# paninski-lab/deepgraphpose

Measured on AMD Instinct MI355X. Metric: frames_per_sec, higher is better.
Workload: dtype f32

## Files before the change

### deepgraphpose_amd/_lib.py

```python
from __future__ import annotations

import ctypes as C
import os

_HERE = os.path.dirname(os.path.abspath(__file__))
LIB_PATH = os.environ.get("DGP_HIP_LIB") or os.path.join(_HERE, "libdgp_hip.so")


class DgpNetDesc(C.Structure):
    _fields_ = [("depth", C.c_int32), ("num_joints", C.c_int32), ("in_h", C.c_int32), ("in_w", C.c_int32),
                ("max_batch", C.c_int32), ("with_locref", C.c_int32), ("mean_pixel", C.c_float * 3),
                ("bn_eps", C.c_float)]


class DgpTensorView(C.Structure):
    _fields_ = [("name", C.c_char_p), ("data", C.POINTER(C.c_float)), ("ndim", C.c_int32),
                ("shape", C.c_int64 * 4)]


class DgpLossDesc(C.Structure):
    _fields_ = [(n, C.c_int32) for n in ("nt", "H", "W", "nj", "nl", "n_visible", "n_hidden", "gm2", "gm3",
                                          "gauss_len", "huber")] + \
               [(n, C.c_float) for n in ("gamma", "lengthscale", "stride", "wn_visible", "wn_hidden",
                                         "locref_loss_weight", "n_frames_total", "n_visible_frames_total")] + \
# ... 8 lines not shown
class DgpJpegInfo(C.Structure):
    _fields_ = [(n, C.c_int32) for n in ("width", "height", "ncomp", "sampling", "mcus_x", "mcus_y")] + \
               [("blocks_x", C.c_int32 * 3), ("blocks_y", C.c_int32 * 3), ("blocks", C.c_int32 * 3)] + \
               [(n, C.c_int32) for n in ("total_blocks", "restart_interval", "reserved")] + [("scan_offset", C.c_int64)]


class DgpConvDesc(C.Structure):
    _fields_ = [(n, C.c_int32) for n in (
        "N", "H", "W", "Cin", "Cout", "KH", "KW", "stride", "rate", "pad_t", "pad_l", "Ho", "Wo", "relu",
        "res_stride", "res_H", "res_W")]


class DgpConvPlan(C.Structure):
    _fields_ = [(n, C.c_int32) for n in (
        "tile", "family", "mode", "cs", "dma", "deep", "ah2", "oh2", "h1", "lds", "mtiles", "ntiles", "grid",
        "tail_ksplit", "n_main", "st_gn", "st_mc", "st_mb", "n_cu")] + [("kernel_name", C.c_char * 32)]


_vp, _i32, _f32, _sz = C.c_void_p, C.c_int32, C.c_float, C.c_size_t
SYMBOLS = {
    "dgp_version": (C.c_int, []),
    "dgp_tuning_build": (C.c_int, []),
    "dgp_crc32c": (C.c_uint32, [C.c_void_p, C.c_size_t, C.c_uint32]),
    "dgp_last_error": (C.c_char_p, []),
    "dgp_net_create": (C.c_int, [C.POINTER(DgpNetDesc), C.POINTER(_vp)]),
    "dgp_net_destroy": (None, [_vp]),
    "dgp_net_set_input_size": (C.c_int, [_vp, _i32, _i32]),
    "dgp_dlc_loss_fwd_bwd": (C.c_int, [_vp, _vp, _vp, _vp, _vp, _vp, _i32, _i32, _i32, _i32, C.c_float, _i32, _vp, _vp, _vp,
                                       _vp, _sz, _vp]),
    "dgp_net_load_weights": (C.c_int, [_vp, C.POINTER(DgpTensorView), _i32]),
    "dgp_net_workspace_bytes": (C.c_int, [_vp, _i32, C.POINTER(_sz)]),
    "dgp_net_output_dims": (C.c_int, [_vp] + [C.POINTER(_i32)] * 4),
    "dgp_net_stats": (C.c_int, [_vp, _i32, C.POINTER(_i32), C.POINTER(C.c_double)]),
    "dgp_forward": (C.c_int, [_vp, _vp, _i32, _vp, _sz, _vp, _vp, _vp, _vp]),
    "dgp_soft_argmax": (C.c_int, [_vp, _i32, _i32, _i32, _i32, _f32, _i32, _vp, _vp, _vp, _vp, _vp]),
    "dgp_soft_argmax_locref": (C.c_int, [_vp, _vp, _i32, _i32, _i32, _i32, _f32, _i32, _vp, _vp, _vp, _vp, _vp, _vp]),
    "dgp_hard_argmax": (C.c_int, [_vp, _vp, _i32, _i32, _i32, _i32, _vp, _vp, _vp, _vp]),
    "dgp_pmap_threshold": (C.c_int, [_vp, _i32, _i32, _i32, _i32, _f32, _vp, _vp]),
    "dgp_infer": (C.c_int, [_vp, _vp, _i32, _vp, _sz, _f32, _i32, _vp, _vp, _vp, _vp, _vp]),
    "dgp_infer_packed": (C.c_int, [_vp, _vp, _i32, _vp, _sz, _f32, _i32, _vp, _vp, _vp]),
    "dgp_infer_packed_locref": (C.c_int, [_vp, _vp, _i32, _vp, _sz, _f32, _i32, _i32, _vp, _vp, _vp, _vp]),
    "dgp_net_profile_begin": (C.c_int, [_vp, _i32]),
    "dgp_net_profile_end": (C.c_int, [_vp, C.POINTER(_i32), C.POINTER(_i32)]),
    "dgp_net_profile_launch": (C.c_int, [_vp, _i32, C.c_char_p, _i32, C.POINTER(C.c_double), C.POINTER(C.c_double)]),
    "dgp_loss_scratch_bytes": (C.c_int, [C.POINTER(DgpLossDesc), C.POINTER(_sz)]),
    "dgp_loss_fwd_bwd": (C.c_int, [C.POINTER(DgpLossDesc)] + [_vp] * 18 + [_sz, _vp]),
    "dgp_trainer_create": (C.c_int, [_vp, C.POINTER(_vp)]),
    "dgp_trainer_destroy": (None, [_vp]),
    "dgp_trainer_num_tensors": (C.c_int, [_vp, C.POINTER(_i32), C.POINTER(C.c_int64), C.POINTER(C.c_int64)]),
    "dgp_trainer_tensor_info": (C.c_int, [_vp, _i32, C.c_char_p, _i32, C.POINTER(C.c_int64), C.POINTER(C.c_int64),
                                          C.POINTER(_i32)]),
    "dgp_trainer_buffer": (_vp, [_vp, _i32]),
    "dgp_trainer_upload": (C.c_int, [_vp, _i32, C.c_int64, _vp, C.c_int64]),
    "dgp_trainer_download": (C.c_int, [_vp, _i32, C.c_int64, _vp, C.c_int64]),
    "dgp_trainer_workspace_bytes": (C.c_int, [_vp, _i32, C.POINTER(_sz)]),
    "dgp_trainer_sync_weights": (C.c_int, [_vp, _vp]),
    "dgp_train_forward": (C.c_int, [_vp, _vp, _i32, _vp, _sz, C.POINTER(_vp), C.POINTER(_vp), _vp]),
    "dgp_train_backward": (C.c_int, [_vp, _i32, _vp, _sz, _vp, _vp, _vp]),
    "dgp_sgd_momentum_clip": (C.c_int, [_vp, _f32, _f32, _f32, C.POINTER(_f32), _vp]),
    "dgp_adam_clip": (C.c_int, [_vp, _f32, _f32, _f32, _f32, _f32, C.POINTER(_f32), _vp]),
    "dgp_packed_weight_floats": (_sz, [_i32, _i32, _i32, _i32]),
    "dgp_pack_conv_weights": (C.c_int, [_vp, _i32, _i32, _i32, _i32, _vp]),
    "dgp_conv2d": (C.c_int, [C.POINTER(DgpConvDesc), _vp, _vp, _vp, _vp, _vp, _vp, _vp]),
    "dgp_conv2d_ranged": (C.c_int, [C.POINTER(DgpConvDesc), _vp, _vp, _vp, _vp, _vp, _vp, _vp, _vp, _vp, _vp]),
    "dgp_conv2d_ranged_slab": (C.c_int, [C.POINTER(DgpConvDesc), _vp, _vp, _vp, _vp, _vp, _vp, _vp, _vp, _vp, _vp, _sz, _vp]),
    "dgp_conv2d_plan": (C.c_int, [C.POINTER(DgpConvDesc), _i32, _i32, _i32, _i32, _i32, _sz, _i32, _i32, C.POINTER(DgpConvPlan)]),
    "dgp_tensor_absmax": (C.c_int, [_vp, _sz, _vp, _vp]),
    "dgp_f32_to_h2": (C.c_int, [_vp, _sz, _i32, _vp, _vp]),
    "dgp_h2_to_f32": (C.c_int, [_vp, _sz, _i32, _vp, _vp]),
    "dgp_conv2d_h2": (C.c_int, [C.POINTER(DgpConvDesc), _vp, _i32, _vp, _vp, _vp, _vp, _vp, _i32, _i32, _vp, _i32, _i32, _vp, _vp, _vp]),
    "dgp_conv2d_h2_slab": (C.c_int, [C.POINTER(DgpConvDesc), _vp, _i32, _vp, _vp, _vp, _vp, _vp, _i32, _i32, _vp, _i32, _i32, _vp, _vp, _vp,
                                     _sz, _vp]),
    "dgp_net_set_tier": (C.c_int, [_vp, _i32]),
    "dgp_net_get_tier": (C.c_int, [_vp]),
    "dgp_f32_to_h1": (C.c_int, [_vp, _sz, _i32, _vp, _vp]),
    "dgp_h1_to_f32": (C.c_int, [_vp, _sz, _i32, _vp, _vp]),
    "dgp_conv2d_h1": (C.c_int, [C.POINTER(DgpConvDesc), _vp, _i32, _vp, _vp, _vp, _vp, _vp, _i32, _vp, _i32, _i32, _vp, _vp, _vp]),
    "dgp_chain_h2": (C.c_int, [_i32] * 9 + [_vp, _i32, _vp, _i32] + [_vp] * 6 + [_vp, _i32, _vp, _i32, _vp, _vp, _vp]),
    "dgp_unit_h2": (C.c_int, [_i32] * 7 + [_vp, _i32, _vp, _i32] + [_vp] * 3 + [_i32] + [_vp] * 6 + [_vp, _i32, _vp, _i32, _vp, _vp, _vp, _vp]),
    "dgp_chain_h1": (C.c_int, [_i32] * 9 + [_vp, _i32, _vp, _i32] + [_vp] * 6 + [_vp, _i32, _vp, _i32, _vp, _vp, _vp]),
    "dgp_unit_h1": (C.c_int, [_i32] * 7 + [_vp, _i32, _vp, _i32] + [_vp] * 3 + [_i32] + [_vp] * 6 + [_vp, _i32, _vp, _i32, _vp, _vp, _vp, _vp]),
    "dgp_chain_xkeep": (C.c_int, [_i32] * 11 + [_vp, _i32, _vp, _i32] + [_vp] * 6 + [_vp, _i32, _vp, _i32, _vp, _vp, _vp]),
    "dgp_unit_xkeep": (C.c_int, [_i32] * 9 + [_vp, _i32, _vp, _i32] + [_vp] * 3 + [_i32] + [_vp] * 6 + [_vp, _i32, _vp, _i32, _vp, _vp, _vp, _vp]),
    "dgp_net_range_status": (C.c_int, [_vp, C.POINTER(_i32), C.POINTER(_i32), _vp]),
    "dgp_net_recalibrate": (C.c_int, [_vp]),
    "dgp_net_reset_scales": (C.c_int, [_vp]),
    "dgp_net_copy_scales": (C.c_int, [_vp, _vp, _vp]),
    "dgp_net_widen": (C.c_int, [_vp]),
    "dgp_conv2d_wgrad": (C.c_int, [C.POINTER(DgpConvDesc), _vp, _vp, _vp, _vp, _vp, _vp, _vp]),
    "dgp_conv2d_wgrad_shadow": (C.c_int, [C.POINTER(DgpConvDesc), _vp, _vp, _vp, _vp, _vp, _vp, _vp, _vp, _vp, _vp]),
    "dgp_trainer_set_tier": (C.c_int, [_vp, C.c_int32]),
    "dgp_trainer_get_tier": (C.c_int, [_vp]),
    "dgp_trainer_grad_groups": (C.c_int, [_vp, C.c_int32, C.POINTER(C.c_int32), C.POINTER(C.c_int64), C.POINTER(C.c_int64)]),
    "dgp_trainer_grad_group_wait": (C.c_int, [_vp, C.c_int32, _vp]),
    "dgp_trainer_step_status": (C.c_int, [_vp, _vp, C.c_int32, C.POINTER(C.c_float), C.POINTER(C.c_float), C.POINTER(C.c_int32),
                                               C.POINTER(C.c_int32), _vp]),
    "dgp_trainer_fast_mode": (C.c_int, [_vp, C.c_int32]),
    "dgp_trainer_fast_status": (C.c_int, [_vp, C.POINTER(C.c_int32), C.POINTER(C.c_int32)]),
    "dgp_conv2d_dgrad_scratch_bytes": (_sz, [C.POINTER(DgpConvDesc)]),
    "dgp_conv2d_dgrad": (C.c_int, [C.POINTER(DgpConvDesc), _vp, _vp, _vp, _vp, _vp, _i32, _vp, _vp, _i32, _vp]),
    "dgp_h1_to_f32_pred": (C.c_int, [_vp, _sz, _vp, _vp, _vp, _vp]),
    "dgp_conv2d_wgrad_h1": (C.c_int, [C.POINTER(DgpConvDesc)] + [_vp] * 11),
    "dgp_conv2d_dgrad_h1": (C.c_int, [C.POINTER(DgpConvDesc), _vp, _vp, _vp, _vp, _vp, _i32] + [_vp] * 7),
    "dgp_stem_wgrad_h1": (C.c_int, [_vp] * 4 + [_i32] * 7 + [_vp] * 4),
    "dgp_heads_backward_h1": (C.c_int, [_vp] * 8 + [_i32] * 5 + [_vp] * 8),
    "dgp_motion_energy":(C.c_int, [_vp, C.c_int64, C.c_int32, _vp, _vp, _vp]),
    "dgp_maxpool_3x3s2_same": (C.c_int, [_vp, _i32, _i32, _i32, _i32, _vp, _vp]),
    "dgp_preprocess_u8": (C.c_int, [_vp, C.c_int64, C.POINTER(_f32), _vp, _vp]),
    "dgp_optical_flow_scratch_bytes": (C.c_int, [_i32, _i32, _i32, C.POINTER(DgpFlowParams), C.POINTER(_sz), C.POINTER(_i32)]),
    "dgp_optical_flow": (C.c_int, [_vp, _i32, _i32, _i32, C.POINTER(DgpFlowParams), _vp, _vp, _vp, _sz, _vp]),
    "dgp_resize_plan_size": (C.c_int, [_i32, _i32, C.POINTER(_i32)]),
    "dgp_resize_plan": (C.c_int, [_i32, _i32, _vp, _vp]),
    "dgp_resize_crop_u8": (C.c_int, [_vp, _i32, _i32, _i32, _i32, _i32, C.POINTER(_i32), _vp, _vp, _vp, _i32, _i32, _vp]),
    "dgp_resize_plan_size_f": (C.c_int, [_i32, _i32, _i32, C.POINTER(_i32)]),
    "dgp_resize_plan_f": (C.c_int, [_i32, _i32, _i32, _vp, _vp]),
    "dgp_window_resize_u8": (C.c_int, [_vp, _i32, _i32, _i32, _i32, _i32, _i32, _i32, _i32, _i32, _i32, _vp, _vp, _vp, _i32, _i32, _vp]),
    "dgp_target_maps": (C.c_int, [_vp, _vp, _vp, _vp, _i32, _i32, _i32, _i32, C.c_double, C.c_double, C.c_double, C.c_double, _i32,
                                  _vp, _vp, _vp, _vp, _vp]),
    "dgp_gather_frames_u8": (C.c_int, [_vp, C.c_int64, C.c_int64, _vp, _i32, _vp, _i32, C.c_int64, _vp, _vp]),
    "dgp_aug_affine_u8": (C.c_int, [_vp, _vp, _i32, _i32, C.POINTER(C.c_double), _vp]),
    "dgp_aug_blur3_u8": (C.c_int, [_vp, _vp, _i32, _i32, C.POINTER(_f32), _vp]),
    "dgp_aug_dropout_u8": (C.c_int, [_vp, _vp, _i32, _i32, _vp, _i32, _i32, _vp]),
    "dgp_aug_elastic_u8": (C.c_int, [_vp, _vp, _i32, _i32, _vp, _i32, _i32, _vp]),
    "dgp_aug_noise_u8": (C.c_int, [_vp, _vp, _i32, _i32, _f32, _i32, C.c_uint64, _vp]),
    "dgp_jpeg_probe": (C.c_int, [_vp, C.c_int64, C.POINTER(DgpJpegInfo)]),
    "dgp_jpeg_entropy_decode": (C.c_int, [_vp, C.c_int64, C.POINTER(DgpJpegInfo), _vp, _vp]),
    "dgp_jpeg_scratch_bytes": (_sz, [_i32, _i32, _i32, _i32]),
    "dgp_jpeg_reconstruct_u8": (C.c_int, [_vp, _vp, _i32, _i32, _i32, _i32, _vp, C.c_int64, _vp, _sz, _vp]),
    "dgp_jpeg_quality_tables": (C.c_int, [_i32, _vp]),
    "dgp_jpeg_encode_bound": (C.c_int64, [_i32, _i32, _i32]),
    "dgp_jpeg_entropy_encode": (C.c_int, [_vp, _i32, _i32, _i32, _vp, _vp, C.c_int64, C.POINTER(C.c_int64)]),
    "dgp_jpeg_forward_scratch_bytes": (_sz, [_i32, _i32, _i32, _i32]),
    "dgp_jpeg_forward_u8": (C.c_int, [_vp, _i32, _i32, _i32, C.c_int64, _i32, _vp, _vp, _i32, _i32, _vp, _vp, _sz, _vp]),
}

_lib = None


class DgpError(RuntimeError):
    pass


def load():
    global _lib
    if _lib is not None:
        return _lib
    if not os.path.exists(LIB_PATH):
        raise DgpError(
            "libdgp_hip.so not found at %s -- build it with `python -m deepgraphpose_amd.build` "
            "(hipcc --offload-arch=gfx950); deepgraphpose_amd has no CPU fallback" % LIB_PATH)
    try:
        import torch
    except ImportError:
        pass
    lib = C.CDLL(LIB_PATH)
    for name, (res, args) in SYMBOLS.items():
        fn = getattr(lib, name)
        fn.restype = res
        fn.argtypes = args
    _lib = lib
    return lib


def check(rc: int, what: str = ""):
    if rc != 0:
        msg = load().dgp_last_error()
# ... 2 lines not shown
```

### deepgraphpose_amd/arch.py

```python
from __future__ import annotations

import math
from dataclasses import dataclass
from typing import List, Tuple

BLOCKS = {
    50: [(64, 3, 2), (128, 4, 2), (256, 6, 2), (512, 3, 1)],
    101: [(64, 3, 2), (128, 4, 2), (256, 23, 2), (512, 3, 1)],
    152: [(64, 3, 2), (128, 8, 2), (256, 36, 2), (512, 3, 1)],
}

MEAN_PIXEL = (123.68, 116.779, 103.939)
BN_EPS = 1e-5


@dataclass
class UnitPlan:
    scope: str
    depth_in: int
    depth: int
    depth_bottleneck: int
    stride: int
    rate: int
    has_shortcut_conv: bool


def resnet_units(depth: int = 50, output_stride: int = 16) -> List[UnitPlan]:
    if depth not in BLOCKS:
        raise ValueError("unsupported resnet depth %r" % (depth,))
    name = "resnet_v1_%d" % depth
    target = output_stride // 4
    current_stride, rate = 1, 1
    units: List[UnitPlan] = []
    depth_in = 64
    for bi, (base, n_units, block_stride) in enumerate(BLOCKS[depth], start=1):
        for ui in range(1, n_units + 1):
            s = block_stride if ui == n_units else 1
            d_out = base * 4
            if current_stride == target:
                unit_stride, unit_rate = 1, rate
                rate *= s
            else:
                unit_stride, unit_rate = s, 1
                current_stride *= s
            units.append(UnitPlan(
                scope="%s/block%d/unit_%d/bottleneck_v1" % (name, bi, ui),
                depth_in=depth_in, depth=d_out, depth_bottleneck=base,
                stride=unit_stride, rate=unit_rate,
                has_shortcut_conv=(depth_in != d_out)))
            depth_in = d_out
    return units


def same_out(n: int, s: int) -> int:
    return -(-n // s)


def feature_hw(h: int, w: int, depth: int = 50) -> Tuple[int, int]:
    for _ in range(4):
        h, w = same_out(h, 2), same_out(w, 2)
    return h, w


def scoremap_hw(h: int, w: int, deconv_stride: int = 2) -> Tuple[int, int]:
    fh, fw = feature_hw(h, w)
    return fh * deconv_stride, fw * deconv_stride


def conv_macs_per_frame(h: int, w: int, depth: int = 50, nj: int = 4,
                        with_locref: bool = False) -> int:
    h1, w1 = same_out(h, 2), same_out(w, 2)
    macs = h1 * w1 * 7 * 7 * 3 * 64
    hh, ww = same_out(h1, 2), same_out(w1, 2)
    for u in resnet_units(depth):
        ho, wo = same_out(hh, u.stride), same_out(ww, u.stride)
        if u.has_shortcut_conv:
            macs += ho * wo * u.depth_in * u.depth
        macs += hh * ww * u.depth_in * u.depth_bottleneck
        macs += ho * wo * 9 * u.depth_bottleneck * u.depth_bottleneck
        macs += ho * wo * u.depth_bottleneck * u.depth
        hh, ww = ho, wo
    heads = nj * (3 if with_locref else 1)
    macs += hh * ww * 9 * 2048 * heads
    return macs


def launch_algorithmic_bytes(name: str, h: int, w: int, depth: int = 50, batch: int = 1, elem_bytes: float = 4.0) -> float:
    body = name.split("|")[0]
    if not body.startswith("conv:"):
        return 0.0
    if body.endswith("/conv1+pool"):
        h1, w1 = same_out(h, 2), same_out(w, 2)
        return float(batch * h * w * 3 + elem_bytes * batch * same_out(h1, 2) * same_out(w1, 2) * 64 + 4 * 7 * 7 * 3 * 64)
    toks = body[5:].split("+")
    units = {u.scope: (i, u) for i, u in enumerate(resnet_units(depth))}
    plan = resnet_units(depth)
    h1, w1 = same_out(h, 2), same_out(w, 2)
    hh, ww = same_out(h1, 2), same_out(w1, 2)
    geo = []
    for u in plan:
        ho, wo = same_out(hh, u.stride), same_out(ww, u.stride)
        geo.append((batch * hh * ww, batch * ho * wo))
        hh, ww = ho, wo
    convs = []
    for t in toks:
        if t == "shortcut":
            convs.append((convs[-1][0], "shortcut"))
            continue
        scope, _, which = t.rpartition("/")
        if scope not in units:
            return 0.0
        convs.append((units[scope][0], which))
    have = set(convs)
    total = 0.0
    for ui, which in convs:
        u = plan[ui]
        pin, pout = geo[ui]
        if which == "conv1":
            total += u.depth_in * u.depth_bottleneck
            total += pin * u.depth_bottleneck
            if (ui - 1, "conv3") not in have:
                total += pin * u.depth_in
        elif which == "conv2":
            total += 9 * u.depth_bottleneck * u.depth_bottleneck
            total += pin * u.depth_bottleneck
            if (ui, "conv3") not in have:
                total += pout * u.depth_bottleneck
        elif which == "conv3":
            total += u.depth_bottleneck * u.depth
            un = plan[ui + 1] if ui + 2 < len(plan) else None
            if (ui + 1, "conv1") in have and un is not None and un.stride == 2 and not un.has_shortcut_conv:
                pin_n, pout_n = geo[ui + 1]
                assert pin_n == pout
                total += pout_n * u.depth
            else:
                total += pout * u.depth
            if (ui, "conv2") not in have:
                total += pout * u.depth_bottleneck
            if (ui, "shortcut") in have:
                total += pin * u.depth_in
            elif u.has_shortcut_conv:
                total += pout * u.depth
            else:
                total += (pin if u.stride == 1 else pout) * u.depth
        elif which == "shortcut":
            total += u.depth_in * u.depth
            if (ui, "conv3") not in have:
                total += pin * u.depth_in + pout * u.depth
    return elem_bytes * total


def conv_algorithmic_bytes(h: int, w: int, depth: int = 50, batch: int = 1) -> dict:
    name = "resnet_v1_%d" % depth
    out = {}
    h1, w1 = same_out(h, 2), same_out(w, 2)
    out["conv:%s/conv1" % name] = 4.0 * (batch * h * w * 4 + batch * h1 * w1 * 64 + 7 * 7 * 4 * 64)
    hh, ww = same_out(h1, 2), same_out(w1, 2)
    for u in resnet_units(depth):
        ho, wo = same_out(hh, u.stride), same_out(ww, u.stride)
        pin, pout = batch * hh * ww, batch * ho * wo
        if u.has_shortcut_conv:
            out["conv:%s/shortcut" % u.scope] = 4.0 * (pin * u.depth_in + pout * u.depth + u.depth_in * u.depth)
        out["conv:%s/conv1" % u.scope] = 4.0 * (pin * u.depth_in + pin * u.depth_bottleneck + u.depth_in * u.depth_bottleneck)
        out["conv:%s/conv2" % u.scope] = 4.0 * (pin * u.depth_bottleneck + pout * u.depth_bottleneck +
                                                9 * u.depth_bottleneck * u.depth_bottleneck)
        res = pout * u.depth if u.has_shortcut_conv else (pin if u.stride == 1 else pout) * u.depth
        out["conv:%s/conv3" % u.scope] = 4.0 * (pout * u.depth_bottleneck + pout * u.depth + res + u.depth_bottleneck * u.depth)
        hh, ww = ho, wo
    return out
```

### deepgraphpose_amd/csrc/dgp_engine.h

```cpp
#pragma once
#include "../../include/dgp_hip.h"
#include "dgp_internal.h"

#include <cmath>
#include <cstdio>
#include <cstring>
#include <initializer_list>
#include <map>
#include <string>
#include <vector>

namespace dgp {
int fail(int code, const std::string& msg);
}
#define HIP_TRY(expr)                                                                          \
    do {                                                                                       \
        hipError_t _e = (expr);                                                                \
        if (_e != hipSuccess)                                                                  \
            return dgp::fail(DGP_ERR_HIP, std::string(#expr) + ": " + hipGetErrorString(_e));  \
    } while (0)

namespace dgp {

struct ConvLayer {
    std::string scope;
    int Cin = 0, Cout = 0, CoutP = 0, KH = 1, KW = 1, stride = 1, rate = 1;
    int nk = 0, ntaps = 1;
    bool has_bn = true, relu = false;
    float *d_w = nullptr, *d_scale = nullptr, *d_bias = nullptr;
    void* d_wh3 = nullptr;
    void* d_wh1 = nullptr;
    float *d_w_fused = nullptr, *d_bias_fused = nullptr;
    void* d_wh3_fused = nullptr;
    void* d_wh1_fused = nullptr;
    int nk_fused = 0, cin2 = 0;
    float* d_w_rows = nullptr;
    float* d_w_pw = nullptr;
    void* d_wh3_pw = nullptr;
    void* d_wh1_pw = nullptr;
    int coutp_pw = 0;
};

struct Unit {
    int sc = -1, c1 = -1, c2 = -1, c3 = -1;
    int stride = 1, rate = 1;
    int depth_in = 0, depth = 0, depth_bn = 0;
    int h = 0, w = 0, ho = 0, wo = 0, pb_h = 0, pb_w = 0;
};

struct ChainPlan {
    bool ok = false;
    int C = 0, C1 = 0, CIN2 = 0, res = 0;
    void* d_frags = nullptr;
    unsigned frag_bytes = 0;
    float *d_sc1 = nullptr, *d_bi1 = nullptr;
    int w3_exp = 0, w1_exp = 0;
    bool unit = false;
    int w2_exp = 0;
    unsigned head_bytes = 0;
    void* d_frags_h1 = nullptr;
    unsigned frag_bytes_h1 = 0, head_bytes_h1 = 0;
};
int build_chain_plan(ChainPlan& pl, int C, int C1, int CIN2, int res, const float* w3cat, const float* sc3, const float* bi3,
                     const float* w1, const float* sc1, const float* bi1, const float* w2 = nullptr, const float* sc2 = nullptr,
                     const float* bi2 = nullptr);
void free_chain_plan(ChainPlan& pl);

constexpr size_t TAIL_SLAB_FLOATS = (size_t)512 * 128 * 128;

int coutp_for(int cout);
int head_pw_coutp(int cpw);
int nk_for(int kh, int kw, int cin);
void tf_same(int n, int k, int s, int d, int* out, int* pad_before);
int pad_before_for(int n, int k, int stride, int rate, bool conv2d_same_explicit);

inline bool fits_descriptor(std::initializer_list<double> bytes) {
    for (double b : bytes) if (b > 4294967000.0) return false;
    return true;
}

inline int fill_conv_geometry(ConvArgs& a, const dgp_conv_desc& d, const char* too_big) {
    a.N = d.N; a.H = d.H; a.W = d.W; a.Cin = d.Cin; a.log2cin4 = ilog2(d.Cin / 4);
    a.Ho = d.Ho; a.Wo = d.Wo; a.Cout = d.Cout; a.CoutP = coutp_for(d.Cout);
    a.KH = d.KH; a.KW = d.KW; a.stride = d.stride; a.dil = d.rate; a.pad_t = d.pad_t; a.pad_l = d.pad_l;
    a.ntaps = d.KH * d.KW; a.nk = nk_for(d.KH, d.KW, d.Cin); a.M = d.N * d.Ho * d.Wo;
    a.res_s = d.res_stride; a.res_H = d.res_H; a.res_W = d.res_W; a.relu = d.relu;
    const double inb = (double)d.N * d.H * d.W * d.Cin * 4, outb = (double)a.M * d.Cout * 4;
    const double resb = a.res ? (double)d.N * d.res_H * d.res_W * d.Cout * 4 : 0.0;
    if (!fits_descriptor({inb, outb, resb})) return fail(DGP_ERR_INVALID, too_big);
    a.in_bytes = (unsigned)inb; a.out_bytes = (unsigned)outb; a.res_bytes = (unsigned)resb;
    a.w_bytes = (unsigned)((size_t)a.nk * 8 * a.CoutP * 16);
    return DGP_OK;
}
const char* const TOO_BIG = "activation tensor exceeds the 4 GiB buffer-descriptor range; lower the batch";

inline ConvArgs head_pointwise_args(const ConvLayer& l, const float* feat, int B, int h, int w, float* T, const float* feat_absmax,
                                    const float* w_absmax) {
    ConvArgs a{};
    a.in = feat; a.wpk = l.d_w_pw; a.wh3 = l.d_wh3_pw; a.out = T; a.in_absmax = feat_absmax; a.w_absmax = w_absmax;
    a.N = B; a.H = h; a.W = w; a.Cin = l.Cin; a.log2cin4 = ilog2(l.Cin / 4);
    a.Ho = h; a.Wo = w; a.Cout = l.coutp_pw; a.CoutP = l.coutp_pw;
    a.KH = 1; a.KW = 1; a.stride = 1; a.dil = 1; a.ntaps = 1; a.nk = nk_for(1, 1, l.Cin); a.M = B * h * w;
    a.in_bytes = (unsigned)((size_t)a.M * l.Cin * 4); a.out_bytes = (unsigned)((size_t)a.M * l.coutp_pw * 4);
    a.w_bytes = (unsigned)((size_t)a.nk * 8 * l.coutp_pw * 16); a.wh3_bytes = a.w_bytes;
    return a;
}

}

struct dgp_net {
    dgp_net_desc desc{};
    int device = 0;
    std::vector<dgp::ConvLayer> layers;
    int conv1 = -1, head_part = -1, head_locref = -1;
    std::vector<dgp::Unit> units;
    std::vector<dgp::ChainPlan> chains;
    bool loaded = false;
    int (*owner_sync)(void* owner, void* stream) = nullptr;
    void* owner = nullptr;
    int tier = 0;
    int h1 = 0, w1 = 0, hp = 0, wp = 0, fh = 0, fw = 0;
    float *d_wmax = nullptr, *d_amax = nullptr, *d_inmax = nullptr;
    float* tail_slab = nullptr;
    unsigned tail_slab_bytes = 0;
    bool wmax_valid = false;
    static constexpr int H2_NONE = (int)0x80000000;
    std::vector<int> act_exp;
    std::vector<char> unit_fuse_ok;
    bool h2_calibrated = false;
    int h2_head = 4;
    int h2_calibrations = 0;
    int *d_exps = nullptr, *d_flag = nullptr;
    const float* wmax(int li) const { return d_wmax ? d_wmax + (size_t)li * dgp::ABSMAX_SLOTS : nullptr; }
    float* amax(int li) const { return d_amax ? d_amax + (size_t)li * dgp::ABSMAX_SLOTS : nullptr; }
    bool prof_on = false, prof_in_infer = false;
    int prof_slots = 0, prof_used = 0, prof_launches = 0, prof_cursor = 0, prof_launches_used = 0;
    std::vector<hipEvent_t> prof_ev;
    std::vector<std::string> prof_names;
    std::vector<double> prof_flops;
    void prof_free() {
        for (auto e : prof_ev) (void)hipEventDestroy(e);
        prof_ev.clear();
    }
    ~dgp_net() {
        prof_free();
        for (auto& l : layers) {
            if (l.d_w) (void)hipFree(l.d_w);
            if (l.d_scale) (void)hipFree(l.d_scale);
            if (l.d_bias) (void)hipFree(l.d_bias);
            if (l.d_wh3) (void)hipFree(l.d_wh3);
            if (l.d_w_rows) (void)hipFree(l.d_w_rows);
            if (l.d_w_pw) (void)hipFree(l.d_w_pw);
            if (l.d_wh3_pw) (void)hipFree(l.d_wh3_pw);
            for (void* q : {l.d_wh1, l.d_wh1_fused, l.d_wh1_pw}) if (q) (void)hipFree(q);
            for (void* q : {(void*)l.d_w_fused, (void*)l.d_bias_fused, l.d_wh3_fused}) if (q) (void)hipFree(q);
        }
        for (auto& c : chains) dgp::free_chain_plan(c);
        for (float* q : {d_wmax, d_amax, d_inmax}) if (q) (void)hipFree(q);
        for (int* q : {d_exps, d_flag}) if (q) (void)hipFree(q);
    }
};
```

### deepgraphpose_amd/csrc/dgp_internal.h

```cpp
#pragma once
#include <hip/hip_runtime.h>
#include <stdint.h>
#include <stddef.h>
#include <stdlib.h>
#include <string.h>

namespace dgp {

constexpr int BK = 32;

struct ConvArgs {
    const float* in;
    const float* wpk;
    const float* scale;
    const float* bias;
    const float* res;
    const float* mask;
    float*       out;
    int N, H, W, Cin, log2cin4;
    int Ho, Wo, Cout, CoutP;
    int KH, KW, stride, dil, pad_t, pad_l;
    int ntaps, nk;
    int M;
    int res_s, res_H, res_W;
    int ksplit;
    long long split_stride;
    int up;
    int relu;
    int out_mode;
    int dc_nj;
    int mtiles, ntiles;
    int tap_minor;
    int stem;
    int tap_rows;
    float* slab;
    unsigned slab_bytes;
    int n_main, tail_ksplit;
    int epi_nt;
    int st_gn, st_mc, st_mb;
    const float* in2;
    const float* in2_absmax;
    unsigned in2_bytes;
    int cin_split;
    unsigned long long* dbg;
    unsigned in_bytes, w_bytes, res_bytes, out_bytes;
    const float* in_absmax;
    const float* w_absmax;
    const void*  wh3;
    unsigned     wh3_bytes;
    float*       out_absmax;
    int   in_fmt, out_fmt, res_fmt;
    float in_scale;
    float out_scale;
    float res_inv_scale;
    float*       shadow;
    const float* shadow_prev;
    int          shadow_fmt;
    const float* in_scale_dev;
    const float* out_scale_dev;
    const float* res_scale_dev;
    int mask_fmt;
};

constexpr int ABSMAX_SLOTS = 256;

enum TileCfg { TILE_128x128 = 0, TILE_128x64 = 1, TILE_64x64 = 2, TILE_128x32 = 3, TILE_128x128_W8 = 4, TILE_128x128_LS = 5, TILE_128x64_LS = 6, TILE_128x128_S6 = 7, TILE_128x128_S3 = 8, TILE_128x64_S6 = 9, TILE_128x128_S6K16 = 10, TILE_128x128_S3K16 = 11, TILE_128x128_S6K16W8 = 12, TILE_128x128_H3K16 = 13, TILE_128x128_H3K16W8 = 14, TILE_128x64_H3 = 15, TILE_128x128_H3K32 = 16 };

enum TileFamily { FAM_F32, FAM_LS, FAM_SPLIT };

struct SplitPath {
    int mode;
    bool pb;
    bool cs, dma, deep;
    bool ah2, oh2, h1;
    size_t lds;
};

struct ConvPlan {
    int tile;
    TileFamily family;
    bool wide;
    SplitPath path;
    int mtiles, ntiles;
    long long grid;
    int tail_ksplit, n_main;
    int st_gn, st_mc, st_mb;
};
hipError_t plan_conv(ConvArgs& a, int tile_cfg, int n_cu, ConvPlan& pl);
hipError_t launch_conv(const ConvArgs& a, int tile_cfg, hipStream_t s);
int        pick_tile(int M, int CoutP, int K, bool have_absmax = false);
hipError_t launch_pack_h3(const float* panel, int nk, int CoutP, const float* w_absmax, void* out, hipStream_t s);
hipError_t launch_pack_h1(const float* panel, int nk, int CoutP, const float* w_absmax, void* out, hipStream_t s);
hipError_t launch_f32_to_h1(const float* x, long long n_groups8, float scale, void* out, hipStream_t s);
hipError_t launch_h1_to_f32(const void* x, long long n_groups8, float inv_scale, float* out, hipStream_t s);
struct PackH3Desc { const float* panel; int nkg; int CoutP; const float* rng; void* out; };
hipError_t launch_pack_h3_all(const PackH3Desc* table_dev, int n, hipStream_t s);
hipError_t launch_pack_h1_all(const PackH3Desc* table_dev, int n, hipStream_t s);
hipError_t launch_absmax(const float* x, long long n, float* out_slots, hipStream_t s);
const char* conv_kernel_name(const ConvArgs& a, int tile_cfg);
hipError_t launch_reduce_slabs(const float* slabs, long long n, long long stride, int nsplit, float* out, hipStream_t s);
hipError_t launch_head_gather(const float* T, const float* bias, int B, int h, int w, int njt, int ldt, float* out, hipStream_t s);
hipError_t launch_maxpool(const float* x, int N, int H, int W, int C, float* y, hipStream_t s, float h2_scale = 0.f);
hipError_t launch_f32_to_h2(const float* x, long long n_groups8, float scale, void* out, hipStream_t s);
hipError_t launch_h2_to_f32(const void* x, long long n_groups8, float inv_scale, float* out, hipStream_t s);
hipError_t launch_h2_range_check(const float* amax_slots, const int* exps, int n_layers, int* flag, hipStream_t s);
hipError_t launch_stem_pool_fused(const unsigned char* frames, int B, int H, int W, const void* wcells, const float* w_absmax,
                                  const float* bn_scale, const float* bn_bias, float m0, float m1, float m2, float out_scale,
                                  float* out, float* out_absmax, hipStream_t s, int out_h1 = 0, const float* out_prev = nullptr,
                                  unsigned char* idx = nullptr);
hipError_t launch_preprocess(const uint8_t* f, long long npix, float m0, float m1, float m2,
                             float* out, hipStream_t s);
hipError_t launch_motion_energy(const uint8_t* frames, long long frame_bytes, int n_frames, const uint8_t* prev_frame,
                                unsigned long long* sums, hipStream_t s);
constexpr size_t SOFT_ARGMAX_LDS_LIMIT = 150 * 1024;
hipError_t launch_soft_argmax(const float* scmap, int B, int H, int W, int C, float gamma,
                              int gauss_len, float* mu, float* conf, int* idx, float* pmap,
                              hipStream_t s, int record_stride = 0);
hipError_t launch_soft_argmax_locref(const float* scmap, const float* locref, int B, int H, int W, int C, float gamma,
                                     int gauss_len, float* mu, float* conf, int* idx, float* offs, float* pmap,
                                     hipStream_t s, int record_stride = 0);
hipError_t launch_hard_argmax(const float* scmap, const float* locref, int B, int H, int W, int C,
                              int* idx, float* prob, float* offs, hipStream_t s, float* rec = nullptr, int record_stride = 0);
hipError_t launch_pmap_threshold(float* pmap, int B, int H, int W, int C, float th, float* mu, hipStream_t s);

struct LossArgs {
    const float* pred;
    const float* locref_pred;
    const float* mu;
    const float* targets;
    const float* locref_map;
    const float* locref_mask;
    const int* visible_marker; const int* hidden_marker; const int* visible_in_targets;
    const float* S0; const float* ws; const float* ws_max;
    float* dpred; float* dlocref;
    float* losses;
    float* t_all; float* dLdt; int* kind; float* stats; float* norm;
    int nt, H, W, nj, nl, n_v, n_h;
    int gm2, gm3, gauss_len, huber;
    float gamma, lengthscale, stride, hidden_scale, clique_scale, locref_weight;
    const float* vector_field; const float* wt_batch; float* wt_w;
    int use_wt, Hin, Win;
    float wt_max, temporal_scale;
};
constexpr size_t LOSS_LDS_LIMIT = 150 * 1024;
hipError_t launch_loss(const LossArgs& a, hipStream_t s);

struct DlcLossArgs {
    const float *pred, *part_targets, *part_weights;
    const float *locref_pred, *locref_targets, *locref_mask;
    float *dpred, *dlocref, *losses;
    double* acc;
    long long n_part, n_loc;
    float locref_loss_weight;
    int huber;
};
hipError_t launch_dlc_loss(const DlcLossArgs& a, hipStream_t s);

struct ChainArgs {
    const void* r2;
    const void* src2;
    void* xout;
    void* r1out;
    const void* wfrag;
    const float* sc1;
    const float* bi1;
    float post1, post2;
    float res_inv_scale, xout_scale, r1_scale;
    float* xout_absmax; float* r1_absmax;
    int M, HoWo, Wo, res_H, res_W;
    int ntiles;
    unsigned r2_bytes, src2_bytes, xout_bytes, r1_bytes, w_bytes;
    const void* r1in;
    unsigned r1in_bytes;
    int H, W, TY, TX;
    float post0, r2_scale;
    float* r2_absmax;
    int nt;
    int h1;
    int xkeep;
};
bool chain_supported(int C, int C1, int CIN2, int res);
int  chain_frags_per_chunk(int C, int C1, int CIN2, int planes = 2);
hipError_t launch_chain(const ChainArgs& a, int C, int C1, int CIN2, int res, hipStream_t s);
const char* chain_kernel_name(int C, int C1, int CIN2, int res);
bool unit_supported(int C, int C1, int CIN2, int res);
hipError_t launch_unit(const ChainArgs& a, int N, int C, int C1, int CIN2, int res, hipStream_t s);
hipError_t launch_chain_pack(const float* src, int n_chunks, int f1_pairs, int f2_pairs, float s1, float s2, void* out, hipStream_t s, int planes = 2);

inline int dgp_env(const char* name, int dflt) {
    const char* v = getenv(name);
    return v ? atoi(v) : dflt;
}
// ... 46 lines not shown
```

### deepgraphpose_amd/csrc/dgp_net.hip

```cpp
#include "dgp_engine.h"

using namespace dgp;

static thread_local std::string g_err;
namespace dgp {
int fail(int code, const std::string& msg) {
    g_err = msg;
    return code;
}

int coutp_for(int cout) {
    if (cout <= 32) return 32;
    if (cout <= 64) return 64;
    return round_up(cout, 128);
}
int head_pw_coutp(int cpw) { const int c = coutp_for(cpw); return c < 64 ? 64 : c; }
int nk_for(int kh, int kw, int cin) { return (kh * kw * (cin / 4) + 7) / 8; }

void tf_same(int n, int k, int s, int d, int* out, int* pad_before) {
    const int keff = (k - 1) * d + 1;
    *out = (n + s - 1) / s;
    int total = (*out - 1) * s + keff - n;
    if (total < 0) total = 0;
    *pad_before = total / 2;
// ... 19 lines not shown

int build_chain_plan(ChainPlan& pl, int C, int C1, int CIN2, int res, const float* w3cat, const float* sc3, const float* bi3,
                     const float* w1, const float* sc1, const float* bi1, const float* w2, const float* sc2, const float* bi2) {
    free_chain_plan(pl);
    if (!chain_supported(C, C1, CIN2, res)) return DGP_OK;
    const bool unit = w2 && unit_supported(C, C1, CIN2, res);
    const int C4 = 4 * C, KS1 = (C + CIN2) / 32, NJP = C4 / 32, NCB = C1 / 16;
    const int pairs = KS1 * 2 + NCB;
    const size_t chunk_f = (size_t)pairs * 512 + 256;
    const int KS2 = C / 32, NCB2 = C / 16, pairs2 = KS2 * NCB2;
    const size_t chunk2_f = (size_t)pairs2 * 512 + 256;
    std::vector<float> src((size_t)NJP * chunk_f, 0.f), src2(unit ? 9 * chunk2_f : 0, 0.f);
    float m3 = 0.f, m1 = 0.f, m2 = 0.f;
    for (size_t i = 0; i < (size_t)(C + CIN2) * C4; ++i) m3 = std::max(m3, fabsf(w3cat[i]));
    for (size_t i = 0; i < (size_t)C4 * C1; ++i) m1 = std::max(m1, fabsf(w1[i]));
    auto col_of = [](int cb, int i) { return 32 * (cb >> 1) + 8 * (i >> 2) + 4 * (cb & 1) + (i & 3); };
    for (int jp = 0; jp < NJP; ++jp) {
        float* ch = src.data() + (size_t)jp * chunk_f;
        for (int s = 0; s < KS1; ++s)
            for (int b = 0; b < 2; ++b) {
                float* f = ch + (size_t)(s * 2 + b) * 512;
                for (int ln = 0; ln < 64; ++ln) {
                    const int g = ln >> 4, i = ln & 15, col = 32 * jp + col_of(b, i);
                    for (int j = 0; j < 8; ++j) f[ln * 8 + j] = w3cat[(size_t)(32 * s + 8 * g + j) * C4 + col];
                }
            }
        for (int cb = 0; cb < NCB; ++cb) {
            float* f = ch + (size_t)(KS1 * 2 + cb) * 512;
            for (int ln = 0; ln < 64; ++ln) {
                const int g = ln >> 4, i = ln & 15, col = col_of(cb, i);
                for (int j = 0; j < 8; ++j) f[ln * 8 + j] = w1[(size_t)(32 * jp + 8 * g + j) * C1 + col];
            }
        }
        float* af = ch + (size_t)pairs * 512;
        for (int c = 0; c < 32; ++c) { af[c] = sc3 ? sc3[32 * jp + c] : 1.f; af[32 + c] = bi3 ? bi3[32 * jp + c] : 0.f; }
    }
    if (unit) {
        for (size_t i = 0; i < (size_t)9 * C * C; ++i) m2 = std::max(m2, fabsf(w2[i]));
        for (int t = 0; t < 9; ++t) {
            float* ch = src2.data() + (size_t)t * chunk2_f;
            for (int ks = 0; ks < KS2; ++ks)
                for (int cb = 0; cb < NCB2; ++cb) {
                    float* f = ch + (size_t)(ks * NCB2 + cb) * 512;
                    for (int ln = 0; ln < 64; ++ln) {
                        const int g = ln >> 4, i = ln & 15, col = col_of(cb, i);
                        for (int j = 0; j < 8; ++j) f[ln * 8 + j] = w2[((size_t)t * C + 32 * ks + 8 * g + j) * C + col];
                    }
                }
            float* af = ch + (size_t)pairs2 * 512;
            for (int c = 0; c < C; ++c) { af[c] = sc2 ? sc2[c] : 1.f; af[C + c] = bi2 ? bi2[c] : 0.f; }
        }
    }
    pl.C = C; pl.C1 = C1; pl.CIN2 = CIN2; pl.res = res; pl.unit = unit;
    pl.w3_exp = pow2_exp_for_max(m3); pl.w1_exp = pow2_exp_for_max(m1); pl.w2_exp = pow2_exp_for_max(m2);
    const int nf = chain_frags_per_chunk(C, C1, CIN2), nf2 = 2 * pairs2 + 1;
    const size_t head = unit ? (size_t)9 * nf2 * 1024 : 0;
    pl.frag_bytes = (unsigned)(head + (size_t)NJP * nf * 1024);
    pl.head_bytes = (unsigned)head;
    float *d_src = nullptr, *d_src2 = nullptr;
    HIP_TRY(hipMalloc(&d_src, src.size() * sizeof(float)));
    hipError_t e = hipMemcpy(d_src, src.data(), src.size() * sizeof(float), hipMemcpyHostToDevice);
    if (e == hipSuccess) e = hipMalloc(&pl.d_frags, pl.frag_bytes);
    if (e == hipSuccess && unit) e = hipMalloc(&d_src2, src2.size() * sizeof(float));
    if (e == hipSuccess && unit) e = hipMemcpy(d_src2, src2.data(), src2.size() * sizeof(float), hipMemcpyHostToDevice);
    if (e == hipSuccess && unit) e = launch_chain_pack(d_src2, 9, pairs2, 0, ldexpf(1.f, pl.w2_exp), 1.f, pl.d_frags, nullptr);
    if (e == hipSuccess) e = launch_chain_pack(d_src, NJP, KS1 * 2, NCB, ldexpf(1.f, pl.w3_exp), ldexpf(1.f, pl.w1_exp), (char*)pl.d_frags + head, nullptr);
    const int nf_h1 = chain_frags_per_chunk(C, C1, CIN2, 1), nf2_h1 = pairs2 + 1;
    const size_t head_h1 = unit ? (size_t)9 * nf2_h1 * 1024 : 0;
    pl.frag_bytes_h1 = (unsigned)(head_h1 + (size_t)NJP * nf_h1 * 1024);
    pl.head_bytes_h1 = (unsigned)head_h1;
    if (e == hipSuccess) e = hipMalloc(&pl.d_frags_h1, pl.frag_bytes_h1);
    if (e == hipSuccess && unit) e = launch_chain_pack(d_src2, 9, pairs2, 0, ldexpf(1.f, pl.w2_exp), 1.f, pl.d_frags_h1, nullptr, 1);
    if (e == hipSuccess) e = launch_chain_pack(d_src, NJP, KS1 * 2, NCB, ldexpf(1.f, pl.w3_exp), ldexpf(1.f, pl.w1_exp), (char*)pl.d_frags_h1 + head_h1, nullptr, 1);
    if (e == hipSuccess) e = hipDeviceSynchronize();
    (void)hipFree(d_src);
    if (d_src2) (void)hipFree(d_src2);
    if (e == hipSuccess) e = hipMalloc(&pl.d_sc1, C1 * sizeof(float));
    if (e == hipSuccess) e = hipMalloc(&pl.d_bi1, C1 * sizeof(float));
    std::vector<float> one(C1, 1.f), zero(C1, 0.f);
    if (e == hipSuccess) e = hipMemcpy(pl.d_sc1, sc1 ? sc1 : one.data(), C1 * sizeof(float), hipMemcpyHostToDevice);
    if (e == hipSuccess) e = hipMemcpy(pl.d_bi1, bi1 ? bi1 : zero.data(), C1 * sizeof(float), hipMemcpyHostToDevice);
    if (e != hipSuccess) { free_chain_plan(pl); return fail(DGP_ERR_HIP, std::string("chain plan: ") + hipGetErrorString(e)); }
    pl.ok = true;
    return DGP_OK;
}
}

namespace {

void pack_panels(const float* hwio, int KH, int KW, int Cin, int Cout, float* packed, int coutp = 0) {
    const int cin4 = Cin / 4, CoutP = coutp ? coutp : coutp_for(Cout), nk = nk_for(KH, KW, Cin);
    const size_t total = (size_t)nk * 8 * CoutP * 4;
    memset(packed, 0, total * sizeof(float));
    const int nchunks = KH * KW * cin4;
    for (int q = 0; q < nchunks; ++q) {
        const int tap = q / cin4, ch = (q % cin4) * 4;
        for (int e = 0; e < 4; ++e) {
            const float* src = hwio + ((size_t)tap * Cin + ch + e) * Cout;
            float* dst = packed + (size_t)q * CoutP * 4 + e;
            for (int co = 0; co < Cout; ++co) dst[(size_t)co * 4] = src[co];
        }
    }
}

}

static int add_layer(dgp_net* net, const std::string& scope, int cin, int cout, int k, int stride, int rate,
                     bool bn, bool relu) {
    ConvLayer l;
    l.scope = scope; l.Cin = cin; l.Cout = cout; l.KH = l.KW = k; l.stride = stride; l.rate = rate;
    l.CoutP = coutp_for(cout); l.nk = nk_for(k, k, cin); l.ntaps = k * k; l.has_bn = bn; l.relu = relu;
    net->layers.push_back(l);
    return (int)net->layers.size() - 1;
}

static void set_geometry(dgp_net* net, int in_h, int in_w) {
    int pb;
    net->desc.in_h = in_h; net->desc.in_w = in_w;
    net->h1 = (in_h + 1) / 2; net->w1 = (in_w + 1) / 2;
    tf_same(net->h1, 3, 2, 1, &net->hp, &pb); tf_same(net->w1, 3, 2, 1, &net->wp, &pb);
    int h = net->hp, w = net->wp;
    for (Unit& u : net->units) {
        u.h = h; u.w = w; tf_same(h, 3, u.stride, u.rate, &u.ho, &pb); tf_same(w, 3, u.stride, u.rate, &u.wo, &pb);
        u.pb_h = pad_before_for(h, 3, u.stride, u.rate, true); u.pb_w = pad_before_for(w, 3, u.stride, u.rate, true);
        h = u.ho; w = u.wo;
    }
    net->fh = h; net->fw = w;
}

extern "C" {

int dgp_version(void) { return DGP_ABI_VERSION; }

uint32_t dgp_crc32c(const void* data, size_t n, uint32_t crc) {
    static uint32_t tab[8][256];
    static bool init = false;
    if (!init) {
        for (uint32_t i = 0; i < 256; ++i) {
            uint32_t c = i;
            for (int k = 0; k < 8; ++k) c = (c & 1) ? (c >> 1) ^ 0x82F63B78u : c >> 1;
            tab[0][i] = c;
        }
        for (uint32_t i = 0; i < 256; ++i)
            for (int t = 1; t < 8; ++t) tab[t][i] = (tab[t - 1][i] >> 8) ^ tab[0][tab[t - 1][i] & 0xFF];
        init = true;
    }
    const uint8_t* p = (const uint8_t*)data;
    crc = ~crc;
    while (n >= 8) {
        uint32_t lo, hi;
        memcpy(&lo, p, 4);
        memcpy(&hi, p + 4, 4);
        lo ^= crc;
        crc = tab[7][lo & 0xFF] ^ tab[6][(lo >> 8) & 0xFF] ^ tab[5][(lo >> 16) & 0xFF] ^ tab[4][lo >> 24] ^
              tab[3][hi & 0xFF] ^ tab[2][(hi >> 8) & 0xFF] ^ tab[1][(hi >> 16) & 0xFF] ^ tab[0][hi >> 24];
        p += 8;
        n -= 8;
    }
    while (n--) crc = tab[0][(crc ^ *p++) & 0xFF] ^ (crc >> 8);
    return ~crc;
}
const char* dgp_last_error(void) { return g_err.c_str(); }
int dgp_tuning_build(void) {
#ifdef DGP_TUNING
    return 1;
#else
// ... 202 lines not shown
            HIP_TRY(hipMemcpy(l.d_w_rows, rows.data(), rows.size() * sizeof(float), hipMemcpyHostToDevice));
            if (!l.d_wh3) HIP_TRY(hipMalloc(&l.d_wh3, rows.size() * sizeof(float)));
            e = launch_pack_h3(l.d_w_rows, 7, l.CoutP, net->d_wmax + li * ABSMAX_SLOTS, l.d_wh3, nullptr);
            if (e != hipSuccess) return fail(DGP_ERR_HIP, std::string("stem weight cells: ") + hipGetErrorString(e));
        } else if (l.d_w_pw) {
            const int nkpw = nk_for(1, 1, 2048);
            float* wm = net->d_wmax + (nl + li) * ABSMAX_SLOTS;
            e = launch_absmax(l.d_w_pw, (long long)nkpw * 8 * l.coutp_pw * 4, wm, nullptr);
            if (e == hipSuccess) e = launch_pack_h3(l.d_w_pw, nkpw, l.coutp_pw, wm, l.d_wh3_pw, nullptr);
            if (e == hipSuccess && !l.d_wh1_pw) e = hipMalloc(&l.d_wh1_pw, (size_t)nkpw * 8 * l.coutp_pw * 8);
            if (e == hipSuccess) e = launch_pack_h1(l.d_w_pw, nkpw, l.coutp_pw, wm, l.d_wh1_pw, nullptr);
            if (e != hipSuccess) return fail(DGP_ERR_HIP, std::string("head pointwise panel: ") + hipGetErrorString(e));
        } else if (l.Cin >= 32 && l.CoutP % 64 == 0) {
            const size_t bytes = (size_t)l.nk * 8 * l.CoutP * 16;
            if (!l.d_wh3) HIP_TRY(hipMalloc(&l.d_wh3, bytes));
            e = launch_pack_h3(l.d_w, l.nk, l.CoutP, net->d_wmax + li * ABSMAX_SLOTS, l.d_wh3, nullptr);
            if (e == hipSuccess && (l.Cin % 64) == 0 && (l.nk % 2) == 0) {
                if (!l.d_wh1) e = hipMalloc(&l.d_wh1, bytes / 2);
                if (e == hipSuccess) e = launch_pack_h1(l.d_w, l.nk, l.CoutP, net->d_wmax + li * ABSMAX_SLOTS, l.d_wh1, nullptr);
            }
            if (e != hipSuccess) return fail(DGP_ERR_HIP, std::string("weight cells: ") + hipGetErrorString(e));
        }
    }
    for (const Unit& u : net->units) {
        if (u.sc < 0) continue;
        ConvLayer& l3 = net->layers[u.c3];
        const ConvLayer& ls = net->layers[u.sc];
        if (l3.KH != 1 || ls.KH != 1 || ls.stride != 1 || l3.Cin % 32 || ls.Cin % 32 || l3.Cout != ls.Cout) continue;
        const int c1 = l3.Cin, c2 = ls.Cin, co = l3.Cout;
        std::vector<float> w((size_t)(c1 + c2) * co), b(co);
        const std::vector<float>&w3 = keep_w[u.c3], &wsc = keep_w[u.sc], &s3 = keep_scale[u.c3], &ssc = keep_scale[u.sc];
        for (int k = 0; k < c1; ++k) for (int o = 0; o < co; ++o) w[(size_t)k * co + o] = w3[(size_t)k * co + o] * s3[o];
        for (int k = 0; k < c2; ++k) for (int o = 0; o < co; ++o) w[(size_t)(c1 + k) * co + o] = wsc[(size_t)k * co + o] * ssc[o];
        for (int o = 0; o < co; ++o) b[o] = keep_bias[u.c3][o] + keep_bias[u.sc][o];
        l3.nk_fused = (c1 + c2) / 32; l3.cin2 = c2;
        const size_t nfl = (size_t)l3.nk_fused * 8 * l3.CoutP * 4;
        std::vector<float> packed(nfl);
        pack_panels(w.data(), 1, 1, c1 + c2, co, packed.data());
        if (!l3.d_w_fused) HIP_TRY(hipMalloc(&l3.d_w_fused, nfl * sizeof(float)));
        if (!l3.d_bias_fused) HIP_TRY(hipMalloc(&l3.d_bias_fused, co * sizeof(float)));
        if (!l3.d_wh3_fused) HIP_TRY(hipMalloc(&l3.d_wh3_fused, nfl * sizeof(float)));
        HIP_TRY(hipMemcpy(l3.d_w_fused, packed.data(), nfl * sizeof(float), hipMemcpyHostToDevice));
        HIP_TRY(hipMemcpy(l3.d_bias_fused, b.data(), co * sizeof(float), hipMemcpyHostToDevice));
        float* wm = net->d_wmax + (nl + (size_t)u.c3) * ABSMAX_SLOTS;
        hipError_t e = launch_absmax(l3.d_w_fused, (long long)nfl, wm, nullptr);
        if (e == hipSuccess) e = launch_pack_h3(l3.d_w_fused, l3.nk_fused, l3.CoutP, wm, l3.d_wh3_fused, nullptr);
        if (e == hipSuccess && (c1 % 64) == 0 && (c2 % 64) == 0) {
            if (!l3.d_wh1_fused) e = hipMalloc(&l3.d_wh1_fused, nfl * 2);
            if (e == hipSuccess) e = launch_pack_h1(l3.d_w_fused, l3.nk_fused, l3.CoutP, wm, l3.d_wh1_fused, nullptr);
        }
        if (e != hipSuccess) return fail(DGP_ERR_HIP, std::string("fused shortcut panel: ") + hipGetErrorString(e));
    }
    for (auto& c : net->chains) free_chain_plan(c);
    net->chains.assign(net->units.size(), ChainPlan());
    for (size_t ui = 0; ui + 1 < net->units.size(); ++ui) {
        const Unit &u = net->units[ui], &un = net->units[ui + 1];
        const ConvLayer &l3 = net->layers[u.c3], &l1 = net->layers[un.c1];
        if (l3.KH != 1 || l1.KH != 1 || l1.stride != 1 || l3.Cout != 4 * l3.Cin || l1.Cin != l3.Cout) continue;
        const int C = l3.Cin, C1 = l1.Cout;
        static const bool wide_env = (dgp_tune("DGP_CHAIN_WIDE", 0) != 0);
        if (C > 128 && !wide_env) continue;
        const ConvLayer& l2 = net->layers[u.c2];
        const bool c2_plain = l2.KH == 3 && l2.stride == 1 && l2.rate == 1 && l2.Cin == C && l2.Cout == C;
        const float *w2 = c2_plain ? keep_w[u.c2].data() : nullptr, *s2 = c2_plain ? keep_scale[u.c2].data() : nullptr,
                    *b2 = c2_plain ? keep_bias[u.c2].data() : nullptr;
        int rc2;
        if (u.sc >= 0) {
            const ConvLayer& ls = net->layers[u.sc];
            if (ls.stride != 1 || u.stride != 1 || !l3.d_w_fused) continue;
            const int c2 = ls.Cin, co = l3.Cout;
            std::vector<float> w((size_t)(C + c2) * co), b(co);
            const std::vector<float>&w3 = keep_w[u.c3], &wsc = keep_w[u.sc], &s3 = keep_scale[u.c3], &ssc = keep_scale[u.sc];
            for (int k = 0; k < C; ++k) for (int o = 0; o < co; ++o) w[(size_t)k * co + o] = w3[(size_t)k * co + o] * s3[o];
            for (int k = 0; k < c2; ++k) for (int o = 0; o < co; ++o) w[(size_t)(C + k) * co + o] = wsc[(size_t)k * co + o] * ssc[o];
            for (int o = 0; o < co; ++o) b[o] = keep_bias[u.c3][o] + keep_bias[u.sc][o];
            rc2 = build_chain_plan(net->chains[ui], C, C1, c2, 0, w.data(), nullptr, b.data(), keep_w[un.c1].data(),
                                   keep_scale[un.c1].data(), keep_bias[un.c1].data(), w2, s2, b2);
        } else {
            rc2 = build_chain_plan(net->chains[ui], C, C1, 0, u.stride == 1 ? 1 : 2, keep_w[u.c3].data(), keep_scale[u.c3].data(),
                                   keep_bias[u.c3].data(), keep_w[un.c1].data(), keep_scale[un.c1].data(), keep_bias[un.c1].data(), w2, s2, b2);
        }
        if (rc2) return rc2;
    }
    HIP_TRY(hipDeviceSynchronize());
    net->wmax_valid = true;
    net->loaded = true;
    net->h2_calibrated = false;
    net->h2_head = 4;
    net->act_exp.assign(net->layers.size(), 0);
    net->unit_fuse_ok.assign(net->units.size(), 1);
    if (!net->d_exps) HIP_TRY(hipMalloc(&net->d_exps, net->layers.size() * sizeof(int)));
    if (!net->d_flag) { HIP_TRY(hipMalloc(&net->d_flag, 2 * sizeof(int))); HIP_TRY(hipMemset(net->d_flag, 0, 2 * sizeof(int))); }
    return DGP_OK;
}

}

namespace {

constexpr int HEAD_KSPLIT_MAX = 8;

struct Plan {
    size_t off_p0, off_c1, off_x0, off_x1, off_sc, off_r1, off_r2, off_scmap, off_locref, off_slabs, off_tail, total;
};

size_t align256(size_t x) { return (x + 255) / 256 * 256; }

Plan make_plan(const dgp_net* net, int B) {
    const dgp_net_desc& d = net->desc;
    size_t p0 = (size_t)B * d.in_h * d.in_w * 4;
    size_t c1 = (size_t)B * net->h1 * net->w1 * 64;
    size_t x = (size_t)B * net->hp * net->wp * 64, sc = 0, r1 = 0, r2 = 0;
    for (const Unit& u : net->units) {
        r1 = std::max(r1, (size_t)B * u.h * u.w * u.depth_bn);
        r2 = std::max(r2, (size_t)B * u.ho * u.wo * u.depth_bn);
        x = std::max(x, (size_t)B * u.ho * u.wo * u.depth);
        if (u.sc >= 0) sc = std::max(sc, (size_t)B * u.ho * u.wo * u.depth);
    }
    r1 = r2 = std::max(r1, r2);
    Plan p{};
    size_t o = 0;
    auto take = [&](size_t nfloats) { size_t r = o; o += align256(nfloats * sizeof(float)); return r; };
    p.off_p0 = take(p0); p.off_c1 = take(c1); p.off_x0 = take(x); p.off_x1 = take(x); p.off_sc = take(sc);
    p.off_r1 = take(r1); p.off_r2 = take(r2);
    p.off_scmap = take((size_t)B * 4 * net->fh * net->fw * d.num_joints);
    p.off_locref = take((size_t)B * 4 * net->fh * net->fw * 2 * d.num_joints);
    p.off_slabs = take((size_t)HEAD_KSPLIT_MAX * B * 4 * net->fh * net->fw * 2 * d.num_joints);
    p.off_tail = take(TAIL_SLAB_FLOATS);
    p.total = o;
    return p;
}

struct ProfScope {
    dgp_net* net; hipStream_t s; int li;
    ProfScope(dgp_net* n, hipStream_t st, const std::string& name, double flops) : net(n), s(st), li(-1) {
        if (!net->prof_on || net->prof_used >= net->prof_slots) return;
        li = net->prof_cursor++;
        if (li >= net->prof_launches) { li = -1; return; }
        if (net->prof_used == 0) { net->prof_names[li] = name; net->prof_flops[li] = flops; }
        (void)hipEventRecord(net->prof_ev[((size_t)net->prof_used * net->prof_launches + li) * 2], s);
    }
    ~ProfScope() {
        if (li >= 0) (void)hipEventRecord(net->prof_ev[((size_t)net->prof_used * net->prof_launches + li) * 2 + 1], s);
    }
};

double conv_flops_of(const ConvLayer& l, int M, bool is_head) {
    if (is_head) return 2.0 * M * 9.0 * l.Cin * (l.Cout / 4);
    const int cin = (l.KH == 7) ? 3 : l.Cin;
    return 2.0 * M * (double)l.KH * l.KW * cin * l.Cout;
}

struct H2Spec { int in_fmt = 0, in_exp = 0, out_fmt = 0, out_exp = 0, res_fmt = 0, res_exp = 0; };

void apply_h2(ConvArgs& a, const H2Spec& h) {
    a.in_fmt = h.in_fmt; a.out_fmt = h.out_fmt; a.res_fmt = h.res_fmt;
    a.in_scale = ldexpf(1.f, h.in_exp); a.out_scale = ldexpf(1.f, h.out_exp); a.res_inv_scale = ldexpf(1.f, -h.res_exp);
}

struct ConvCall {
    const float* in = nullptr;
    int H = 0, W = 0, Ho = 0, Wo = 0, pad_t = 0, pad_l = 0;
    const float* res = nullptr;
    int res_s = 0, res_H = 0, res_W = 0;
    bool relu = true;
    int out_mode = 0, dc_nj = 0;
// ... 174 lines not shown
        HIP_TRY(hipStreamSynchronize(s));
        HIP_TRY(hipMemcpy(host, net->amax(li), sizeof host, hipMemcpyDeviceToHost));
        *mx = 0.f;
        for (float v : host) *mx = (v > *mx || v != v) ? v : *mx;
        return DGP_OK;
    }
    template <class Launch>
    int layer(int li, Launch&& launch, int forced_exp = dgp_net::H2_NONE, bool* forced_ok = nullptr) const {
        int r = launch();
        if (r || !calib) return r;
        float mx = 0.f;
        if ((r = read_range(li, &mx))) return r;
        int e = exp_for(mx);
        if (forced_exp != dgp_net::H2_NONE) {
            const bool ok = forced_exp <= e + net->h2_head - 1 && forced_exp >= e - 6;
            if (forced_ok) *forced_ok = ok;
            if (ok) e = forced_exp;
        }
        if (e != net->act_exp[li]) {
            net->act_exp[li] = e;
            HIP_TRY(hipMemsetAsync(net->amax(li), 0, ABSMAX_SLOTS * sizeof(float), s));
            r = launch();
        }
        return r;
    }
    H2Spec spec(int in_exp, int out_li, bool with_res = false, int res_exp = 0) const {
        H2Spec q;
        q.in_fmt = FMT; q.in_exp = in_exp; q.out_fmt = FMT; q.out_exp = net->act_exp[out_li]; q.res_fmt = with_res ? FMT : 0; q.res_exp = res_exp;
        return q;
    }
    bool can_fuse(int ui) const {
        const Unit& u = net->units[ui];
        return fuse_on && u.sc >= 0 && net->layers[u.c3].d_w_fused && u.stride == 1 && u.ho == u.h && u.wo == u.w && net->layers[u.c3].CoutP % 64 == 0;
    }
    int conv(int li, const ConvCall& call) const { return run_conv(net, net->layers[li], B, call, s); }
};

int fwd_context(FwdCtx& c, dgp_net* net, const uint8_t* frames, int B, char* ws, const Plan& pl, hipStream_t s) {
    static const bool h2_env = (dgp_env("DGP_H2", 1) != 0);
    static const bool head_pw = (dgp_tune("DGP_HEAD_PW", 1) != 0);
    static const bool fuse_env = (dgp_env("DGP_FUSE_SHORTCUT", 1) != 0);
    static const bool cells_env = (dgp_tune("DGP_PRESPLIT_WEIGHTS", 1) != 0);
    static const bool stem_fused_env = (dgp_tune("DGP_STEM_FUSED", 1) != 0);
    static const bool chain_env = (dgp_env("DGP_CHAIN", 1) != 0);
    static const bool chain_h1_env = (dgp_env("DGP_CHAIN_H1", 1) != 0);
    static const bool unit_env = (dgp_tune("DGP_UNIT", 1) != 0);
    static const bool xsub_env = (dgp_env("DGP_XOUT_SUBSAMPLE", 1) != 0);
    c = FwdCtx{};
    c.net = net; c.s = s; c.B = B; c.frames = frames;
    c.P0 = (float*)(ws + pl.off_p0); c.C1 = (float*)(ws + pl.off_c1); c.X[0] = (float*)(ws + pl.off_x0); c.X[1] = (float*)(ws + pl.off_x1);
    c.SC = (float*)(ws + pl.off_sc); c.R1 = (float*)(ws + pl.off_r1); c.R2 = (float*)(ws + pl.off_r2);
    c.scmap_ws = (float*)(ws + pl.off_scmap); c.slabs = (float*)(ws + pl.off_slabs);
    const ConvLayer& lpart = net->layers[net->head_part];
    const ConvLayer* lloc = net->head_locref < 0 ? nullptr : &net->layers[net->head_locref];
    c.f16_mode = conv_mode() == ConvMode::F16x3 || conv_mode() == ConvMode::F16;
    c.head_pw = head_pw; c.unit_on = unit_env; c.xsub_on = xsub_env;
    c.fuse_on = fuse_env && conv_mode() != ConvMode::F32 && net->wmax_valid;
    c.tier = net->tier; c.FMT = c.tier ? 2 : 1;
    c.h2 = h2_env && cells_env && c.f16_mode && head_pw && net->wmax_valid && net->d_exps && lpart.d_wh3_pw && (!lloc || lloc->d_wh3_pw) &&
           net->act_exp.size() == net->layers.size();
    if (c.tier) {
        bool ok = c.h2 && lpart.d_wh1_pw && (!lloc || lloc->d_wh1_pw);
        for (const Unit& u : net->units) {
            ok = ok && net->layers[u.c1].d_wh1 && net->layers[u.c2].d_wh1 && net->layers[u.c3].d_wh1 && (u.sc < 0 || net->layers[u.sc].d_wh1);
            if (u.sc >= 0 && net->layers[u.c3].d_w_fused && !net->layers[u.c3].d_wh1_fused) ok = false;
        }
        if (!ok) return fail(DGP_ERR_STATE, "dgp_forward: the 16-bit tier needs the H2 engine's switches at their defaults (DGP_H2, DGP_PRESPLIT_WEIGHTS, "
                                            "DGP_HEAD_PW, DGP_CONV_MODE unset or f16) and weights loaded by dgp_net_load_weights");
    }
    c.calib = c.h2 && !net->h2_calibrated;
    const ConvLayer& lstem = net->layers[net->conv1];
    c.stem_fused = c.h2 && (stem_fused_env || c.tier) && lstem.d_wh3 && lstem.d_w_rows && lstem.CoutP == 64 && lstem.d_scale && lstem.d_bias;
    if (c.tier && !c.stem_fused) return fail(DGP_ERR_STATE, "dgp_forward: the 16-bit tier needs the fused root block");
    c.chain_tier = chain_env && (!c.tier || chain_h1_env);
    c.chain_on = c.h2 && !c.calib && c.chain_tier && net->chains.size() == net->units.size();
    return DGP_OK;
}

int forward_root(FwdCtx& c) {
    dgp_net* net = c.net;
    const dgp_net_desc& d = net->desc;
    const ConvLayer& lstem = net->layers[net->conv1];
    int rc;
    if (c.stem_fused) {
        rc = c.layer(net->conv1, [&] {
            ProfScope ps(net, c.s, "conv:" + lstem.scope + "+pool|stem_pool_fused", conv_flops_of(lstem, c.B * net->h1 * net->w1, false));
            hipError_t e2 = launch_stem_pool_fused(c.frames, c.B, d.in_h, d.in_w, lstem.d_wh3, net->wmax(net->conv1), lstem.d_scale, lstem.d_bias,
                                                   d.mean_pixel[0], d.mean_pixel[1], d.mean_pixel[2],
                                                   ldexpf(1.f, net->act_exp[net->conv1]), c.X[0], net->amax(net->conv1), c.s, c.tier ? 1 : 0);
            return e2 == hipSuccess ? (int)DGP_OK : fail(DGP_ERR_HIP, std::string("stem + pool: ") + hipGetErrorString(e2));
        });
        if (rc) return rc;
    } else {
        hipError_t e;
        {
            ProfScope ps(net, c.s, "preprocess_u8", 0.0);
            e = launch_preprocess(c.frames, (long long)c.B * d.in_h * d.in_w, d.mean_pixel[0], d.mean_pixel[1], d.mean_pixel[2], c.P0, c.s);
        }
        if (e != hipSuccess) return fail(DGP_ERR_HIP, std::string("preprocess: ") + hipGetErrorString(e));
        if ((rc = c.conv(net->conv1, conv_call(c.P0, d.in_h, d.in_w, c.C1).grid(net->h1, net->w1, 3, 3).range(net->d_inmax)))) return rc;
        if (c.calib) {
            float mx = 0.f;
            if ((rc = c.read_range(net->conv1, &mx))) return rc;
            net->act_exp[net->conv1] = c.exp_for(mx);
        }
        {
            ProfScope ps(net, c.s, "maxpool3x3s2", 0.0);
            e = launch_maxpool(c.C1, c.B, net->h1, net->w1, 64, c.X[0], c.s, c.h2 ? ldexpf(1.f, net->act_exp[net->conv1]) : 0.f);
        }
        if (e != hipSuccess) return fail(DGP_ERR_HIP, std::string("maxpool: ") + hipGetErrorString(e));
    }
    c.cur = 0; c.Ra = c.R1; c.Rb = c.R2; c.r1_ready = false;
    c.x_rng = net->amax(net->conv1);
    c.x_exp = c.h2 ? net->act_exp[net->conv1] : 0;
    return DGP_OK;
}

int forward_unit_f32(FwdCtx& c, int ui) {
    dgp_net* net = c.net;
    const Unit& u = net->units[ui];
    const float *xin = c.X[c.cur], *r1_rng = net->amax(u.c1), *r2_rng = net->amax(u.c2);
    float* xout = c.X[c.cur ^ 1];
    const bool fuse = c.can_fuse(ui);
    ConvCall c3 = conv_call(c.R2, u.ho, u.wo, xout).range(r2_rng).residual(xin, u.stride, u.h, u.w);
    int rc = DGP_OK;
    if (u.sc >= 0 && !fuse) {
        rc = c.conv(u.sc, conv_call(xin, u.h, u.w, c.SC).grid(u.ho, u.wo).linear().range(c.x_rng));
        c3.residual(c.SC, 1, u.ho, u.wo);
    }
    if (!rc) rc = c.conv(u.c1, conv_call(xin, u.h, u.w, c.R1).range(c.x_rng));
    if (!rc) rc = c.conv(u.c2, conv_call(c.R1, u.h, u.w, c.R2).grid(u.ho, u.wo, u.pb_h, u.pb_w).range(r1_rng));
    if (!rc) rc = fuse ? run_conv_fused_shortcut(net, u, c.R2, xin, c.B, u.h, u.w, xout, c.s, r2_rng, c.x_rng) : c.conv(u.c3, c3);
    c.x_rng = net->amax(u.c3);
    c.cur ^= 1;
    return rc;
}

int forward_unit_cells(FwdCtx& c, int ui) {
    dgp_net* net = c.net;
    const Unit& u = net->units[ui];
    const float* xin = c.X[c.cur];
    float* xout = c.X[c.cur ^ 1];
    const int x_exp = c.x_exp;
    const bool can_fuse = c.can_fuse(ui);
    bool fuse = can_fuse && (c.calib || net->unit_fuse_ok[ui]);
    int rc;
    if (!c.r1_ready) {
        rc = c.layer(u.c1, [&] { return c.conv(u.c1, conv_call(xin, u.h, u.w, c.Ra).cells(c.spec(x_exp, u.c1))); });
        if (rc) return rc;
    }
    const bool chain_ok = c.chain_on && (size_t)ui + 1 < net->units.size() && net->chains[ui].ok;
    const bool unit_k = chain_ok && c.unit_on && net->chains[ui].unit && (net->chains[ui].res != 0 || fuse);
    bool share_ok = true;
    if (!unit_k) {
        rc = c.layer(u.c2, [&] { return c.conv(u.c2, conv_call(c.Ra, u.h, u.w, c.Rb).grid(u.ho, u.wo, u.pb_h, u.pb_w).cells(c.spec(net->act_exp[u.c1], u.c2))); },
                     (fuse && c.calib) ? x_exp : dgp_net::H2_NONE, &share_ok);
        if (rc) return rc;
    }
    if (c.calib && can_fuse) { net->unit_fuse_ok[ui] = share_ok ? 1 : 0; fuse = share_ok; }
    const bool chain = chain_ok && (net->chains[ui].res != 0 || fuse);
    ConvCall c3 = conv_call(c.Rb, u.ho, u.wo, xout).residual(xin, u.stride, u.h, u.w);
    int res_exp = x_exp;
    if (u.sc >= 0 && !fuse) {
        rc = c.layer(u.sc, [&] { return c.conv(u.sc, conv_call(xin, u.h, u.w, c.SC).grid(u.ho, u.wo).linear().cells(c.spec(x_exp, u.sc))); });
        if (rc) return rc;
        c3.residual(c.SC, 1, u.ho, u.wo);
        res_exp = net->act_exp[u.sc];
    }
    int xkeep = 1;
    if ((unit_k || chain) && c.xsub_on && (size_t)ui + 2 < net->units.size()) {
        const Unit& un = net->units[ui + 1];
        if (un.stride == 2 && un.sc < 0) xkeep = 2;
    }
    if (unit_k) rc = run_chain(net, ui, nullptr, xin, c.B, xout, c.Rb, c.s, x_exp, c.Ra, xkeep);
    else if (chain) rc = run_chain(net, ui, c.Rb, xin, c.B, xout, c.Ra, c.s, x_exp, nullptr, xkeep);
    else if (fuse)
        rc = c.layer(u.c3, [&] { return run_conv_fused_shortcut(net, u, c.Rb, xin, c.B, u.h, u.w, xout, c.s, nullptr, nullptr, c.spec(x_exp, u.c3)); });
    else
        rc = c.layer(u.c3, [&] { return c.conv(u.c3, c3.cells(c.spec(net->act_exp[u.c2], u.c3, true, res_exp))); });
    if (unit_k) std::swap(c.Ra, c.Rb);
    c.r1_ready = unit_k || chain;
    c.x_exp = net->act_exp[u.c3];
    c.x_rng = net->amax(u.c3);
    c.cur ^= 1;
    return rc;
}

int forward_heads(const FwdCtx& c, float* scmap, float* locref, float* features) {
    dgp_net* net = c.net;
    const int B = c.B, h = net->fh, w = net->fw, nj = net->desc.num_joints;
    const float* feat = c.X[c.cur];
    if (features) {
        if (c.h2) {
            const hipError_t e = c.tier ? launch_h1_to_f32(feat, (long long)B * h * w * 2048 / 8, ldexpf(1.f, -c.x_exp), features, c.s)
                                        : launch_h2_to_f32(feat, (long long)B * h * w * 2048 / 8, ldexpf(1.f, -c.x_exp), features, c.s);
// ... 515 lines not shown
    return DGP_OK;
}

struct LayerWeights { const float *w2, *scale2, *bias2, *w3cat, *scale3, *bias3, *w1, *scale1, *bias1; };
static int launch_layer(const std::string& who, const ChainIo& io, int C, int C1, int CIN2, int res_mode, const LayerWeights& w, hipStream_t s) {
    const bool unit = w.w2 != nullptr;
    if (!(unit ? io.r1in : io.r2) || !io.src2 || !w.w3cat || !w.w1 || !io.xout || !io.r1out) return fail(DGP_ERR_INVALID, who + ": null argument");
    if (!(unit ? unit_supported(C, C1, CIN2, res_mode) : chain_supported(C, C1, CIN2, res_mode)))
        return fail(DGP_ERR_INVALID, who + ": no kernel instance for this (C, C1, CIN2, res_mode)");
    if (res_mode == 0 && io.src2_exp != io.r2_exp) return fail(DGP_ERR_INVALID, who + ": the K-concatenated source must share R2's scale");
    if (unit && io.r1in == io.r1out) return fail(DGP_ERR_INVALID, who + ": r1out must not alias r1 (halo reads)");
    ChainPlan cp;
    int rc = build_chain_plan(cp, C, C1, CIN2, res_mode, w.w3cat, w.scale3, w.bias3, w.w1, w.scale1, w.bias1, w.w2, w.scale2, w.bias2);
    if (rc) return rc;
    ChainArgs a{};
    rc = fill_chain_args(a, cp, io);
    hipError_t e = hipSuccess;
    if (!rc) e = unit ? launch_unit(a, io.N, C, C1, CIN2, res_mode, s) : launch_chain(a, C, C1, CIN2, res_mode, s);
    if (!rc && e == hipSuccess) e = hipStreamSynchronize(s);
    free_chain_plan(cp);
    return e != hipSuccess ? fail(DGP_ERR_HIP, who + ": " + hipGetErrorString(e)) : rc;
}

int dgp_chain_h2(int32_t N, int32_t Ho, int32_t Wo, int32_t C, int32_t C1, int32_t CIN2, int32_t res_mode, int32_t res_H, int32_t res_W,
                 const void* r2_h2, int32_t r2_exp, const void* src2_h2, int32_t src2_exp,
                 const float* w3cat, const float* scale3, const float* bias3, const float* w1, const float* scale1, const float* bias1,
                 void* xout_h2, int32_t xout_exp, void* r1_h2, int32_t r1_exp, float* xout_absmax, float* r1_absmax, void* stream) {
    const ChainIo io{false, N, Ho, Wo, res_H, res_W, r2_h2, src2_h2, nullptr, xout_h2, r1_h2, 0, r2_exp, src2_exp, xout_exp, r1_exp,
                     nullptr, xout_absmax, r1_absmax};
    return launch_layer("dgp_chain_h2", io, C, C1, CIN2, res_mode, {nullptr, nullptr, nullptr, w3cat, scale3, bias3, w1, scale1, bias1}, (hipStream_t)stream);
}
int dgp_chain_h1(int32_t N, int32_t Ho, int32_t Wo, int32_t C, int32_t C1, int32_t CIN2, int32_t res_mode, int32_t res_H, int32_t res_W,
                 const void* r2_h1, int32_t r2_exp, const void* src2_h1, int32_t src2_exp,
                 const float* w3cat, const float* scale3, const float* bias3, const float* w1, const float* scale1, const float* bias1,
                 void* xout_h1, int32_t xout_exp, void* r1_h1, int32_t r1_exp, float* xout_absmax, float* r1_absmax, void* stream) {
    const ChainIo io{true, N, Ho, Wo, res_H, res_W, r2_h1, src2_h1, nullptr, xout_h1, r1_h1, 0, r2_exp, src2_exp, xout_exp, r1_exp,
                     nullptr, xout_absmax, r1_absmax};
    return launch_layer("dgp_chain_h1", io, C, C1, CIN2, res_mode, {nullptr, nullptr, nullptr, w3cat, scale3, bias3, w1, scale1, bias1}, (hipStream_t)stream);
}
int dgp_unit_h2(int32_t N, int32_t H, int32_t W, int32_t C, int32_t C1, int32_t CIN2, int32_t res_mode,
                const void* r1_h2, int32_t r1_exp, const void* src2_h2, int32_t src2_exp,
                const float* w2, const float* scale2, const float* bias2, int32_t r2_exp,
                const float* w3cat, const float* scale3, const float* bias3, const float* w1, const float* scale1, const float* bias1,
                void* xout_h2, int32_t xout_exp, void* r1out_h2, int32_t r1out_exp, float* r2_absmax, float* xout_absmax, float* r1_absmax,
                void* stream) {
    if (!w2) return fail(DGP_ERR_INVALID, "dgp_unit_h2: null argument");
    const ChainIo io{false, N, H, W, H, W, nullptr, src2_h2, r1_h2, xout_h2, r1out_h2, r1_exp, r2_exp, src2_exp, xout_exp, r1out_exp,
                     r2_absmax, xout_absmax, r1_absmax};
    return launch_layer("dgp_unit_h2", io, C, C1, CIN2, res_mode, {w2, scale2, bias2, w3cat, scale3, bias3, w1, scale1, bias1}, (hipStream_t)stream);
}
int dgp_unit_h1(int32_t N, int32_t H, int32_t W, int32_t C, int32_t C1, int32_t CIN2, int32_t res_mode,
                const void* r1_h1, int32_t r1_exp, const void* src2_h1, int32_t src2_exp,
                const float* w2, const float* scale2, const float* bias2, int32_t r2_exp,
                const float* w3cat, const float* scale3, const float* bias3, const float* w1, const float* scale1, const float* bias1,
                void* xout_h1, int32_t xout_exp, void* r1out_h1, int32_t r1out_exp, float* r2_absmax, float* xout_absmax, float* r1_absmax,
                void* stream) {
    if (!w2) return fail(DGP_ERR_INVALID, "dgp_unit_h1: null argument");
    const ChainIo io{true, N, H, W, H, W, nullptr, src2_h1, r1_h1, xout_h1, r1out_h1, r1_exp, r2_exp, src2_exp, xout_exp, r1out_exp,
                     r2_absmax, xout_absmax, r1_absmax};
    return launch_layer("dgp_unit_h1", io, C, C1, CIN2, res_mode, {w2, scale2, bias2, w3cat, scale3, bias3, w1, scale1, bias1}, (hipStream_t)stream);
}
int dgp_chain_xkeep(int32_t h1, int32_t xout_keep, int32_t N, int32_t Ho, int32_t Wo, int32_t C, int32_t C1, int32_t CIN2, int32_t res_mode,
                    int32_t res_H, int32_t res_W, const void* r2, int32_t r2_exp, const void* src2, int32_t src2_exp,
                    const float* w3cat, const float* scale3, const float* bias3, const float* w1, const float* scale1, const float* bias1,
                    void* xout, int32_t xout_exp, void* r1, int32_t r1_exp, float* xout_absmax, float* r1_absmax, void* stream) {
    if (xout_keep != 1 && xout_keep != 2) return fail(DGP_ERR_INVALID, "dgp_chain_xkeep: xout_keep must be 1 or 2");
    const ChainIo io{h1 != 0, N, Ho, Wo, res_H, res_W, r2, src2, nullptr, xout, r1, 0, r2_exp, src2_exp, xout_exp, r1_exp,
                     nullptr, xout_absmax, r1_absmax, xout_keep};
    return launch_layer("dgp_chain_xkeep", io, C, C1, CIN2, res_mode, {nullptr, nullptr, nullptr, w3cat, scale3, bias3, w1, scale1, bias1}, (hipStream_t)stream);
}
int dgp_unit_xkeep(int32_t h1, int32_t xout_keep, int32_t N, int32_t H, int32_t W, int32_t C, int32_t C1, int32_t CIN2, int32_t res_mode,
                   const void* r1, int32_t r1_exp, const void* src2, int32_t src2_exp,
                   const float* w2, const float* scale2, const float* bias2, int32_t r2_exp,
                   const float* w3cat, const float* scale3, const float* bias3, const float* w1, const float* scale1, const float* bias1,
                   void* xout, int32_t xout_exp, void* r1out, int32_t r1out_exp, float* r2_absmax, float* xout_absmax, float* r1_absmax,
                   void* stream) {
    if (xout_keep != 1 && xout_keep != 2) return fail(DGP_ERR_INVALID, "dgp_unit_xkeep: xout_keep must be 1 or 2");
    if (!w2) return fail(DGP_ERR_INVALID, "dgp_unit_xkeep: null argument");
    const ChainIo io{h1 != 0, N, H, W, H, W, nullptr, src2, r1, xout, r1out, r1_exp, r2_exp, src2_exp, xout_exp, r1out_exp,
                     r2_absmax, xout_absmax, r1_absmax, xout_keep};
    return launch_layer("dgp_unit_xkeep", io, C, C1, CIN2, res_mode, {w2, scale2, bias2, w3cat, scale3, bias3, w1, scale1, bias1}, (hipStream_t)stream);
}

int dgp_net_range_status(dgp_net* net, int32_t* overflow, int32_t* calibrations, void* stream) {
    if (!net) return fail(DGP_ERR_INVALID, "dgp_net_range_status: null net");
    int flag[2] = {0, 0};
    if (net->d_flag) {
        HIP_TRY(hipStreamSynchronize((hipStream_t)stream));
        HIP_TRY(hipMemcpy(flag, net->d_flag, sizeof flag, hipMemcpyDeviceToHost));
        if (flag[0]) {
            HIP_TRY(hipMemset(net->d_flag, 0, sizeof flag));
            net->h2_calibrated = false;
            net->h2_head = std::min(net->h2_head + 3, 12);
        }
    }
    if (overflow) *overflow = flag[0] ? 1 : 0;
    if (calibrations) *calibrations = net->h2_calibrations;
    return DGP_OK;
}

int dgp_net_recalibrate(dgp_net* net) {
    if (!net) return fail(DGP_ERR_INVALID, "dgp_net_recalibrate: null net");
    net->h2_calibrated = false;
    return DGP_OK;
}

int dgp_net_widen(dgp_net* net) {
    if (!net) return fail(DGP_ERR_INVALID, "dgp_net_widen: null net");
    net->h2_calibrated = false;
    net->h2_head = std::min(net->h2_head + 3, 12);
    return DGP_OK;
}

int dgp_net_copy_scales(dgp_net* dst, const dgp_net* src, void* stream) {
    if (!dst || !src) return fail(DGP_ERR_INVALID, "dgp_net_copy_scales: null net");
    if (!src->h2_calibrated) return fail(DGP_ERR_STATE, "dgp_net_copy_scales: the source engine is not calibrated");
    if (!dst->loaded || !dst->d_exps || dst->layers.size() != src->layers.size() || dst->units.size() != src->units.size() || dst->tier != src->tier ||
        dst->desc.in_h != src->desc.in_h || dst->desc.in_w != src->desc.in_w)
        return fail(DGP_ERR_INVALID, "dgp_net_copy_scales: the engines differ (layers, tier or frame size)");
    dst->act_exp = src->act_exp;
    dst->unit_fuse_ok = src->unit_fuse_ok;
    dst->h2_head = src->h2_head;
    return upload_scales(dst, (hipStream_t)stream);
}

int dgp_net_reset_scales(dgp_net* net) {
    if (!net) return fail(DGP_ERR_INVALID, "dgp_net_reset_scales: null net");
    net->h2_calibrated = false;
    net->h2_head = 4;
    return DGP_OK;
}

int dgp_maxpool_3x3s2_same(const float* x, int32_t N, int32_t H, int32_t W, int32_t C, float* y, void* stream) {
    if (!x || !y || (C & 3)) return fail(DGP_ERR_INVALID, "dgp_maxpool_3x3s2_same: bad argument (C % 4)");
    hipError_t e = launch_maxpool(x, N, H, W, C, y, (hipStream_t)stream);
    if (e != hipSuccess) return fail(DGP_ERR_HIP, std::string("maxpool: ") + hipGetErrorString(e));
    return DGP_OK;
}

int dgp_preprocess_u8(const uint8_t* frames, int64_t n_pixels, const float mean[3], float* out_nhwc4, void* stream) {
    if (!frames || !mean || !out_nhwc4) return fail(DGP_ERR_INVALID, "dgp_preprocess_u8: null argument");
    hipError_t e = launch_preprocess(frames, n_pixels, mean[0], mean[1], mean[2], out_nhwc4, (hipStream_t)stream);
    if (e != hipSuccess) return fail(DGP_ERR_HIP, std::string("preprocess: ") + hipGetErrorString(e));
    return DGP_OK;
}

int dgp_motion_energy(const uint8_t* frames, int64_t frame_bytes, int32_t n_frames, const uint8_t* prev_frame, uint64_t* sums,
                      void* stream) {
    if (!frames || !sums || frame_bytes <= 0 || n_frames <= 0) return fail(DGP_ERR_INVALID, "dgp_motion_energy: bad argument");
    hipError_t e = launch_motion_energy(frames, frame_bytes, n_frames, prev_frame, (unsigned long long*)sums, (hipStream_t)stream);
    if (e != hipSuccess) return fail(DGP_ERR_HIP, std::string("motion energy: ") + hipGetErrorString(e));
    return DGP_OK;
}

}
```

### deepgraphpose_amd/csrc/dgp_ops.hip

```cpp
#include "dgp_internal.h"
#include "dgp_device.h"
#include <cstdlib>
#include <cstring>
#include <cstdio>
#include <vector>
#include <type_traits>

namespace dgp {

__global__ __launch_bounds__(256) void pack_h3_kernel(const float4* __restrict__ panel, int nkg, int CoutP,
                                                      const float* __restrict__ w_absmax, uint4* __restrict__ out) {
    const float s = pow2_scale_for(w_absmax, threadIdx.x & 63);
    const long long total = (long long)nkg * CoutP;
    for (long long g = (long long)blockIdx.x * blockDim.x + threadIdx.x; g < total; g += (long long)gridDim.x * blockDim.x) {
        const int col = (int)(g % CoutP);
        const long long kg = g / CoutP;
        uint2 h0, l0, h1, l1;
        split2_f16(panel[(2 * kg) * CoutP + col], s, h0, l0);
        split2_f16(panel[(2 * kg + 1) * CoutP + col], s, h1, l1);
        out[(kg * 2) * CoutP + col] = make_uint4(h0.x, h0.y, h1.x, h1.y);
        out[(kg * 2 + 1) * CoutP + col] = make_uint4(l0.x, l0.y, l1.x, l1.y);
    }
}

// ... 294 lines not shown
}
constexpr int MEU = 4;
template <int VEC>
__global__ __launch_bounds__(256) void motion_energy_kernel(const uint8_t* __restrict__ frames, long long frame_bytes, int n_frames,
                                                            const uint8_t* __restrict__ prev_frame,
                                                            unsigned long long* __restrict__ sums) {
    const long long nu = frame_bytes / VEC;
    const long long u0 = (long long)blockIdx.x * (256 * MEU) + threadIdx.x;
    const int t0 = blockIdx.y * MEG, t1 = min(n_frames, t0 + MEG);
    const uint8_t* pf = t0 > 0 ? frames + (long long)(t0 - 1) * frame_bytes : prev_frame;
    auto load = [&](const uint8_t* f, int k) {
        const long long u = u0 + 256 * k;
        uint4 v = make_uint4(0, 0, 0, 0);
        if (u < nu) {
            if (VEC == 16) v = *reinterpret_cast<const uint4*>(f + u * 16);
            else v.x = f[u];
        }
        return v;
    };
    uint4 prev[MEU];
#pragma unroll
    for (int k = 0; k < MEU; ++k) prev[k] = pf ? load(pf, k) : make_uint4(0, 0, 0, 0);
    for (int t = t0; t < t1; ++t) {
        const uint8_t* f = frames + (long long)t * frame_bytes;
        uint4 cur[MEU];
#pragma unroll
        for (int k = 0; k < MEU; ++k) cur[k] = load(f, k);
        unsigned s = 0;
        if (pf) {
#pragma unroll
            for (int k = 0; k < MEU; ++k) {
                s = bytes_sub_sum(cur[k].x, prev[k].x, s);
                if (VEC == 16) {
                    s = bytes_sub_sum(cur[k].y, prev[k].y, s); s = bytes_sub_sum(cur[k].z, prev[k].z, s);
                    s = bytes_sub_sum(cur[k].w, prev[k].w, s);
                }
            }
        }
#pragma unroll
        for (int k = 0; k < MEU; ++k) prev[k] = cur[k];
#pragma unroll
        for (int o = 32; o > 0; o >>= 1) s += __shfl_xor(s, o, 64);
        if ((threadIdx.x & 63) == 0 && s) atomicAdd(sums + t, (unsigned long long)s);
        pf = f;
    }
}

hipError_t launch_motion_energy(const uint8_t* frames, long long frame_bytes, int n_frames, const uint8_t* prev_frame,
                                unsigned long long* sums, hipStream_t s) {
    hipError_t e = hipMemsetAsync(sums, 0, (size_t)n_frames * sizeof(unsigned long long), s);
    if (e != hipSuccess) return e;
    const bool vec = (frame_bytes & 15) == 0 && (((uintptr_t)frames | (uintptr_t)prev_frame) & 15) == 0;
    const long long units = vec ? frame_bytes >> 4 : frame_bytes;
    const dim3 grid((unsigned)((units + 256 * MEU - 1) / (256 * MEU)), (unsigned)((n_frames + MEG - 1) / MEG));
    if (vec) hipLaunchKernelGGL(motion_energy_kernel<16>, grid, dim3(256), 0, s, frames, frame_bytes, n_frames, prev_frame, sums);
    else hipLaunchKernelGGL(motion_energy_kernel<1>, grid, dim3(256), 0, s, frames, frame_bytes, n_frames, prev_frame, sums);
    return hipGetLastError();
}

__device__ __forceinline__ float wave_max(float v) {
#pragma unroll
    for (int o = 32; o > 0; o >>= 1) v = fmaxf(v, __shfl_xor(v, o, 64));
    return v;
}
__device__ __forceinline__ double wave_sum(double v) {
#pragma unroll
    for (int o = 32; o > 0; o >>= 1) v += __shfl_xor(v, o, 64);
    return v;
}

struct StemPoolArgs {
    const unsigned char* frames;
    int fr_delta, fr_bytes;
    const uint4* wcells;
    const float* w_absmax;
    const float* bn_scale; const float* bn_bias;
    float mean0, mean1, mean2, out_scale;
    float* out;
    float* out_absmax;
    int out_h1;
    const float* out_prev;
    unsigned char* idx;
    int B, H, W, H1, W1, HP, WP, pbh, pbw, tiles_h, tiles_w, ntiles;
};

template <bool H1T>
__global__ __launch_bounds__(512, 2) void stem_pool_fused_kernel(const StemPoolArgs p) {
    constexpr int PH = H1T ? 3 : 5, PW = 16, SR = 2 * PH + 1, SC = 2 * PW + 1, MS = SR * SC, NRB = (MS + 15) / 16;
    constexpr int IR = 2 * SR + 5, IC = 72;
    static_assert(NRB <= 24 && NRB > 8, "one to three row blocks per wave");
    constexpr int NPL = H1T ? 1 : 2;
    constexpr int WCELLS = 7 * 4 * NPL * 64;
    constexpr int LDC = 68;
    constexpr int LDH = 72;
    typedef float floatx4 __attribute__((ext_vector_type(4)));
    extern __shared__ __attribute__((aligned(16))) char smem[];
    uint4* sW = reinterpret_cast<uint4*>(smem);
    char* sU = smem + WCELLS * 16;
    uint2* sHi = reinterpret_cast<uint2*>(sU);
    constexpr bool ALIAS = !H1T;
    float* sC = reinterpret_cast<float*>(sU + (ALIAS ? 0 : IR * IC * 8));
    _Float16* sCh = reinterpret_cast<_Float16*>(sU + IR * IC * 8);
    const int t = threadIdx.x, lane = t & 63, wave = __builtin_amdgcn_readfirstlane(t >> 6);
    const int l15 = lane & 15, g = lane >> 4;
    for (int i = t; i < WCELLS; i += 512) {
        if constexpr (H1T) sW[i] = p.wcells[((i >> 6) * 2) * 64 + 4 * (i & 15) + ((i >> 4) & 3)];
        else sW[i] = p.wcells[i];
    }
    const float post = 1.f / pow2_scale_for(p.w_absmax, lane);
    const float oscale = p.out_prev ? shadow_scale_for(p.out_prev, lane) : p.out_scale;
    const int nrb = (NRB - wave + 7) / 8;
    float sc4[4][1], bi4[4][1];
#pragma unroll
    for (int j = 0; j < 4; ++j) {
        const int ch = H1T ? 4 * l15 + j : 16 * j + l15;
        sc4[j][0] = p.bn_scale[ch] * post; bi4[j][0] = p.bn_bias[ch];
    }
    float amax = 0.f;
    constexpr int NG = IC / 4;
    static_assert(IC % 4 == 0 && IR * NG <= 512, "one group per thread");
    const int fr_r = t / NG, fr_c = 4 * (t - fr_r * NG);
    const bool fr_on = t < IR * NG;
    const __amdgpu_buffer_rsrc_t rs_fr = __builtin_amdgcn_make_buffer_rsrc(const_cast<unsigned char*>(p.frames), 0, p.fr_bytes & ~3, 0x00020000);
    unsigned pix[3] = {0u, 0u, 0u};
    auto fetch = [&](int tile) {
        const int n = tile / (p.tiles_h * p.tiles_w), rem = tile - n * (p.tiles_h * p.tiles_w);
        const int ir0 = 2 * (2 * (rem / p.tiles_w) * PH - p.pbh) - 3, ic0 = 2 * (2 * (rem % p.tiles_w) * PW - p.pbw) - 3;
        const int gr = ir0 + fr_r, gc = ic0 + fr_c;
        if (!fr_on || (unsigned)gr >= (unsigned)p.H) return;
        const int start = ((n * p.H + gr) * p.W + gc) * 3 + p.fr_delta;
        if (gc >= 0 && (start & ~3) + 16 <= (p.fr_bytes & ~3)) {
            const u32x4 d = __builtin_amdgcn_raw_buffer_load_b128(rs_fr, start & ~3, 0, 0);
            const unsigned sh = (unsigned)start & 3u;
            pix[0] = __builtin_amdgcn_alignbyte(d[1], d[0], sh);
            pix[1] = __builtin_amdgcn_alignbyte(d[2], d[1], sh);
            pix[2] = __builtin_amdgcn_alignbyte(d[3], d[2], sh);
        } else {
            unsigned b[12];
#pragma unroll
            for (int k = 0; k < 4; ++k)
#pragma unroll
                for (int c = 0; c < 3; ++c) b[3 * k + c] = (gc + k >= 0 && start + 3 * k + c < p.fr_bytes) ? (unsigned)p.frames[start + 3 * k + c] : 0u;
#pragma unroll
            for (int w = 0; w < 3; ++w) pix[w] = b[4 * w] | (b[4 * w + 1] << 8) | (b[4 * w + 2] << 16) | (b[4 * w + 3] << 24);
        }
    };
    if ((int)blockIdx.x < p.ntiles) fetch(blockIdx.x);
    for (int tile = blockIdx.x; tile < p.ntiles; tile += gridDim.x) {
        const int n = tile / (p.tiles_h * p.tiles_w), rem = tile - n * (p.tiles_h * p.tiles_w);
        const int ph0 = (rem / p.tiles_w) * PH, pw0 = (rem % p.tiles_w) * PW;
        const int r0 = 2 * ph0 - p.pbh, c0 = 2 * pw0 - p.pbw;
        const int ir0 = 2 * r0 - 3, ic0 = 2 * c0 - 3;
        if (fr_on) {
            const int gr = ir0 + fr_r, gc = ic0 + fr_c;
            const bool rok = (unsigned)gr < (unsigned)p.H;
            unsigned w[8];
#pragma unroll
            for (int k = 0; k < 4; ++k) {
                const unsigned b0 = (pix[(3 * k) >> 2] >> (8 * ((3 * k) & 3))) & 255u, b1 = (pix[(3 * k + 1) >> 2] >> (8 * ((3 * k + 1) & 3))) & 255u,
                               b2 = (pix[(3 * k + 2) >> 2] >> (8 * ((3 * k + 2) & 3))) & 255u;
                half2v x01 = {(_Float16)0.f, (_Float16)0.f}, x23 = x01;
                if (rok && (unsigned)(gc + k) < (unsigned)p.W) {
                    x01 = half2v{(_Float16)((float)b0 - p.mean0), (_Float16)((float)b1 - p.mean1)};
                    x23 = half2v{(_Float16)((float)b2 - p.mean2), (_Float16)1.f};
                }
                w[2 * k] = __builtin_bit_cast(unsigned, x01); w[2 * k + 1] = __builtin_bit_cast(unsigned, x23);
            }
            uint4* dst = reinterpret_cast<uint4*>(sHi + fr_r * IC + fr_c);
            dst[0] = make_uint4(w[0], w[1], w[2], w[3]);
            dst[1] = make_uint4(w[4], w[5], w[6], w[7]);
        }
        __syncthreads();
        if (tile + (int)gridDim.x < p.ntiles) fetch(tile + gridDim.x);
        floatx4 acc[3][4];
#pragma unroll
        for (int i = 0; i < 3; ++i)
#pragma unroll
            for (int j = 0; j < 4; ++j) acc[i][j] = floatx4{0.f, 0.f, 0.f, 0.f};
        int abase[3];
#pragma unroll
        for (int i = 0; i < 3; ++i) {
            int m = 16 * (wave + 8 * i) + l15;
            if (m > MS - 1) m = MS - 1;
            const int rl = m / SC, cl = m - rl * SC;
            abase[i] = (2 * rl) * IC + 2 * cl + 2 * g;
        }
#pragma unroll 1
        for (int kh = 0; kh < 7; ++kh) {
            uint4 bh[4], bl[4];
#pragma unroll
            for (int j = 0; j < 4; ++j) {
                bh[j] = sW[((kh * 4 + g) * NPL + 0) * 64 + 16 * j + l15];
                if constexpr (!H1T) bl[j] = sW[((kh * 4 + g) * NPL + 1) * 64 + 16 * j + l15];
            }
#pragma unroll
            for (int i = 0; i < 3; ++i) {
                if (i < nrb) {
                    const uint4 ah = *reinterpret_cast<const uint4*>(sHi + abase[i] + kh * IC);
#pragma unroll
                    for (int j = 0; j < 4; ++j) {
                        if constexpr (!H1T)
                            acc[i][j] = __builtin_amdgcn_mfma_f32_16x16x32_f16(__builtin_bit_cast(half8, ah), __builtin_bit_cast(half8, bl[j]), acc[i][j], 0, 0, 0);
                        acc[i][j] = __builtin_amdgcn_mfma_f32_16x16x32_f16(__builtin_bit_cast(half8, ah), __builtin_bit_cast(half8, bh[j]), acc[i][j], 0, 0, 0);
                    }
                }
            }
        }
        if constexpr (ALIAS) __syncthreads();
#pragma unroll
        for (int i = 0; i < 3; ++i) {
            if (i < nrb) {
#pragma unroll
                for (int r = 0; r < 4; ++r) {
                    const int m = 16 * (wave + 8 * i) + 4 * g + r;
                    const int rl = m / SC, cl = m - rl * SC;
                    const bool ok = m < MS && (unsigned)(r0 + rl) < (unsigned)p.H1 && (unsigned)(c0 + cl) < (unsigned)p.W1;
                    if constexpr (H1T) {
                        float v4[4];
#pragma unroll
                        for (int j = 0; j < 4; ++j) {
                            v4[j] = ok ? fmaxf(acc[i][j][r] * sc4[j][0] + bi4[j][0], 0.f) : 0.f;
                            amax = fmaxf(amax, v4[j]);
                        }
                        unsigned h01, h23;
                        asm("v_fma_mixlo_f16 %0, %1, %2, 0" : "=v"(h01) : "v"(oscale), "v"(v4[0]));
                        asm("v_fma_mixhi_f16 %0, %1, %2, 0" : "+v"(h01) : "v"(oscale), "v"(v4[1]));
                        asm("v_fma_mixlo_f16 %0, %1, %2, 0" : "=v"(h23) : "v"(oscale), "v"(v4[2]));
                        asm("v_fma_mixhi_f16 %0, %1, %2, 0" : "+v"(h23) : "v"(oscale), "v"(v4[3]));
                        *reinterpret_cast<uint2*>(sCh + m * LDH + 4 * l15) = make_uint2(h01, h23);
                        continue;
                    }
#pragma unroll
                    for (int j = 0; j < 4; ++j) {
                        const float v = fmaxf(acc[i][j][r] * sc4[j][0] + bi4[j][0], 0.f);
                        sC[m * LDC + 16 * j + l15] = ok ? v : 0.f;
                    }
                }
            }
        }
        __syncthreads();
        for (int q = t; q < PH * PW * 8; q += 512) {
            const int pp = q >> 3, cg = q & 7;
            const int ph = pp / PW, pw = pp - ph * PW;
            if constexpr (H1T) {
                half8 mx = {0, 0, 0, 0, 0, 0, 0, 0};
                unsigned kk[8] = {0u, 0u, 0u, 0u, 0u, 0u, 0u, 0u};
                if (p.idx) {
#pragma unroll
                    for (int a = 0; a < 3; ++a)
#pragma unroll
                        for (int b = 0; b < 3; ++b) {
                            const half8 x = *reinterpret_cast<const half8*>(sCh + ((2 * ph + a) * SC + 2 * pw + b) * LDH + 8 * cg);
#pragma unroll
                            for (int k = 0; k < 8; ++k)
                                if (x[k] > mx[k]) { mx[k] = x[k]; kk[k] = (unsigned)(a * 3 + b); }
                        }
                } else {
#pragma unroll
                for (int a = 0; a < 3; ++a)
#pragma unroll
                    for (int b = 0; b < 3; ++b)
                        mx = __builtin_elementwise_max(mx, *reinterpret_cast<const half8*>(sCh + ((2 * ph + a) * SC + 2 * pw + b) * LDH + 8 * cg));
                }
                if (ph0 + ph < p.HP && pw0 + pw < p.WP) {
                    const size_t cell = (((size_t)n * p.HP + ph0 + ph) * p.WP + pw0 + pw) * 8 + cg;
                    if (p.idx)
                        *reinterpret_cast<uint2*>(p.idx + cell * 8) = make_uint2(kk[0] | (kk[1] << 8) | (kk[2] << 16) | (kk[3] << 24),
                                                                                 kk[4] | (kk[5] << 8) | (kk[6] << 16) | (kk[7] << 24));
                    reinterpret_cast<uint4*>(p.out)[cell] = __builtin_bit_cast(uint4, mx);
                }
                continue;
            }
            float v[8];
            unsigned kk[8];
#pragma unroll
            for (int k = 0; k < 8; ++k) { v[k] = 0.f; kk[k] = 0u; }
            if (p.idx) {
#pragma unroll
                for (int a = 0; a < 3; ++a)
#pragma unroll
                    for (int b = 0; b < 3; ++b) {
                        const float* src = sC + ((2 * ph + a) * SC + 2 * pw + b) * LDC + 8 * cg;
                        const float4 x0 = *reinterpret_cast<const float4*>(src), x1 = *reinterpret_cast<const float4*>(src + 4);
                        const float x[8] = {x0.x, x0.y, x0.z, x0.w, x1.x, x1.y, x1.z, x1.w};
#pragma unroll
                        for (int k = 0; k < 8; ++k)
                            if (x[k] > v[k]) { v[k] = x[k]; kk[k] = (unsigned)(a * 3 + b); }
                    }
            } else {
#pragma unroll
            for (int a = 0; a < 3; ++a)
#pragma unroll
                for (int b = 0; b < 3; ++b) {
                    const float* src = sC + ((2 * ph + a) * SC + 2 * pw + b) * LDC + 8 * cg;
                    const float4 x0 = *reinterpret_cast<const float4*>(src), x1 = *reinterpret_cast<const float4*>(src + 4);
                    v[0] = fmaxf(v[0], x0.x); v[1] = fmaxf(v[1], x0.y); v[2] = fmaxf(v[2], x0.z); v[3] = fmaxf(v[3], x0.w);
                    v[4] = fmaxf(v[4], x1.x); v[5] = fmaxf(v[5], x1.y); v[6] = fmaxf(v[6], x1.z); v[7] = fmaxf(v[7], x1.w);
                }
            }
            if (ph0 + ph < p.HP && pw0 + pw < p.WP) {
                uint4 hi, lo;
                h2_pack8(v, oscale, hi, lo);
                const size_t cell = (((size_t)n * p.HP + ph0 + ph) * p.WP + pw0 + pw) * 8 + cg;
                if (p.idx)
                    *reinterpret_cast<uint2*>(p.idx + cell * 8) = make_uint2(kk[0] | (kk[1] << 8) | (kk[2] << 16) | (kk[3] << 24),
                                                                             kk[4] | (kk[5] << 8) | (kk[6] << 16) | (kk[7] << 24));
                uint4* dst = reinterpret_cast<uint4*>(p.out) + (p.out_h1 ? cell : 2 * cell);
                dst[0] = hi;
                if (!p.out_h1) dst[1] = lo;
#pragma unroll
                for (int k = 0; k < 8; ++k) amax = fmaxf(amax, v[k]);
            }
        }
        if constexpr (ALIAS) __syncthreads();
    }
    if (p.out_absmax) track_absmax(p.out_absmax, amax, lane, (int)(blockIdx.x * 8u + (threadIdx.x >> 6)));
}

hipError_t launch_stem_pool_fused(const unsigned char* frames, int B, int H, int W, const void* wcells, const float* w_absmax,
                                  const float* bn_scale, const float* bn_bias, float m0, float m1, float m2, float out_scale,
                                  float* out, float* out_absmax, hipStream_t s, int out_h1, const float* out_prev, unsigned char* idx) {
    if ((long long)B * H * W * 3 >= (1LL << 31)) return hipErrorInvalidValue;
    StemPoolArgs a{};
    a.out_h1 = out_h1; a.out_prev = out_prev; a.idx = idx;
    a.fr_delta = (int)(reinterpret_cast<uintptr_t>(frames) & 3u); a.frames = frames - a.fr_delta; a.fr_bytes = a.fr_delta + B * H * W * 3;
    a.wcells = reinterpret_cast<const uint4*>(wcells); a.w_absmax = w_absmax; a.bn_scale = bn_scale; a.bn_bias = bn_bias;
    a.mean0 = roundf(m0); a.mean1 = roundf(m1); a.mean2 = roundf(m2); a.out_scale = out_scale; a.out = out; a.out_absmax = out_absmax;
    a.B = B; a.H = H; a.W = W; a.H1 = (H + 1) / 2; a.W1 = (W + 1) / 2;
    a.HP = (a.H1 + 1) / 2; a.WP = (a.W1 + 1) / 2;
    const int pth = ((a.HP - 1) * 2 + 3 - a.H1) > 0 ? ((a.HP - 1) * 2 + 3 - a.H1) : 0;
    const int ptw = ((a.WP - 1) * 2 + 3 - a.W1) > 0 ? ((a.WP - 1) * 2 + 3 - a.W1) : 0;
    a.pbh = pth / 2; a.pbw = ptw / 2;
    static const int h1t_env = dgp_tune("DGP_STEM_H1T", 1);
    static const int h1t_train_env = dgp_tune("DGP_STEM_H1T_TRAIN", 1);
    const bool h1t = h1t_env && out_h1 && (!idx || h1t_train_env);
    const int ph = h1t ? 3 : 5;
    a.tiles_h = (a.HP + ph - 1) / ph; a.tiles_w = (a.WP + 15) / 16; a.ntiles = B * a.tiles_h * a.tiles_w;
    const size_t smem = h1t ? (size_t)7 * 4 * 64 * 16 + (size_t)19 * 72 * 8 + (size_t)15 * 16 * 72 * 2 : (size_t)7 * 4 * 2 * 64 * 16 + (size_t)23 * 16 * 68 * 4;
    const hipError_t e = h1t ? ensure_dynamic_lds<stem_pool_fused_kernel<true>>(160 * 1024) : ensure_dynamic_lds<stem_pool_fused_kernel<false>>(160 * 1024);
    if (e != hipSuccess) return e;
    const int n_cu = device_facts().n_cu;
    if (h1t) {
        const int grid = a.ntiles < 2 * n_cu ? a.ntiles : 2 * n_cu;
        hipLaunchKernelGGL(stem_pool_fused_kernel<true>, dim3((unsigned)grid), dim3(512), smem, s, a);
    } else {
        const int grid = a.ntiles < n_cu ? a.ntiles : n_cu;
        hipLaunchKernelGGL(stem_pool_fused_kernel<false>, dim3((unsigned)grid), dim3(512), smem, s, a);
    }
    return hipGetLastError();
}

constexpr int SOFT_ARGMAX_THREADS = 1024;
template <bool LARGE, bool LOCREF>
__global__ __launch_bounds__(SOFT_ARGMAX_THREADS) void soft_argmax_kernel(const float* __restrict__ scmap, int H, int W, int C,
                                                          float gamma, int glen, float* __restrict__ mu,
                                                          float* __restrict__ conf, int* __restrict__ idx,
                                                          float* __restrict__ pmap, int rs,
                                                          const float* __restrict__ locref, float* __restrict__ offs) {
    extern __shared__ __attribute__((aligned(16))) char smem[];
    float* sp = reinterpret_cast<float*>(smem);
    constexpr int NT = SOFT_ARGMAX_THREADS, NW = NT / 64;
    __shared__ double red[LOCREF ? 5 : 3][NW];
    __shared__ float redf[NW];
    __shared__ float gk[16];

    const int b = blockIdx.x / C;
    const int cj = blockIdx.x - b * C;
    const int HW = H * W;
    const float* src = scmap + (long long)b * HW * C + cj;
    const int t = threadIdx.x, lane = t & 63, wave = t >> 6;

    const int r = glen;
    if (t == 0) {
        float s = 0.f;
        for (int i = -r; i <= r; ++i) {
            const float xs = (float)i / (float)glen;
            gk[i + r] = expf(-0.5f * xs * xs);
            s += gk[i + r];
        }
        for (int i = 0; i <= 2 * r; ++i) gk[i] = gk[i] / s;
    }

    auto scaled = [&](int i) -> float { float v = src[(long long)i * C] * gamma; asm volatile("" : "+v"(v)); return v; };
    float mx = -INFINITY;
    for (int i = t; i < HW; i += NT) {
        const float v = scaled(i);
        if (!LARGE) sp[i] = v;
        mx = fmaxf(mx, v);
    }
    mx = wave_max(mx);
    if (lane == 0) redf[wave] = mx;
    __syncthreads();
    mx = redf[0];
#pragma unroll
    for (int k = 1; k < NW; ++k) mx = fmaxf(mx, redf[k]);

    double se = 0.0;
    for (int i = t; i < HW; i += NT) {
        const float e = expf((LARGE ? scaled(i) : sp[i]) - mx);
        if (!LARGE) sp[i] = e;
        se += (double)e;
    }
    se = wave_sum(se);
    if (lane == 0) red[0][wave] = se;
    __syncthreads();
    double dsum = red[0][0];
#pragma unroll
    for (int k = 1; k < NW; ++k) dsum += red[0][k];
    const float denom = (float)dsum;
    __syncthreads();
    if (!LARGE) {
        for (int i = t; i < HW; i += NT) sp[i] = sp[i] / denom;
    }
    __syncthreads();
    auto P = [&](int i) -> float { return LARGE ? expf(scaled(i) - mx) / denom : sp[i]; };

    double s0 = 0.0, sh = 0.0, sw = 0.0, sdx = 0.0, sdy = 0.0;
    for (int i = t; i < HW; i += NT) {
        const int h = i / W, w = i - h * W;
        float acc = 0.f;
        for (int a = -r; a <= r; ++a) {
            const int hh = h + a;
            if ((unsigned)hh >= (unsigned)H) continue;
            const float ga = gk[a + r];
            for (int bb = -r; bb <= r; ++bb) {
                const int ww = w + bb;
                if ((unsigned)ww >= (unsigned)W) continue;
                acc += (ga * gk[bb + r]) * P(hh * W + ww);
            }
        }
// ... 198 lines not shown
```

### deepgraphpose_amd/engine.py

```python
from __future__ import annotations

import ctypes as C
from typing import Dict, NamedTuple, Optional, Tuple

import numpy as np
import torch

from . import _lib
from .arch import MEAN_PIXEL, BN_EPS


def _ptr(t: Optional[torch.Tensor]):
    return None if t is None else C.c_void_p(t.data_ptr())


def _stream(device) -> C.c_void_p:
    return C.c_void_p(torch.cuda.current_stream(device).cuda_stream)


def _need_cuda(t: torch.Tensor, dtype, name: str):
    if not t.is_cuda:
        raise _lib.DgpError("%s must be a device (cuda/HIP) tensor" % name)
    if t.dtype != dtype:
        raise _lib.DgpError("%s must have dtype %s, got %s" % (name, dtype, t.dtype))
# ... 685 lines not shown
    _lib.check(lib.dgp_h2_to_f32(_ptr(x), x.numel(), int(scale_exp), _ptr(out), _stream(x.device)), "dgp_h2_to_f32")
    return out


def conv2d_h2(x_h2: torch.Tensor, x_exp: int, w_hwio: np.ndarray, stride: int = 1, rate: int = 1, pad_t: int = 0, pad_l: int = 0,
              out_hw: Optional[Tuple[int, int]] = None, scale=None, bias=None, residual: Optional[torch.Tensor] = None,
              res_stride: int = 0, res_is_h2: bool = False, res_exp: int = 0, relu: bool = False, y_is_h2: bool = True,
              y_exp: int = 0, tail_slab: Optional[torch.Tensor] = None, out: Optional[torch.Tensor] = None):
    lib = _lib.load()
    _need_cuda(x_h2, torch.float32, "x_h2")
    N, H, W, Cin = x_h2.shape
    kh, kw, cin2, cout = w_hwio.shape
    assert cin2 == Cin
    dev = x_h2.device
    if out_hw is None:
        keh, kew = (kh - 1) * rate + 1, (kw - 1) * rate + 1
        out_hw = ((H + 2 * pad_t - keh) // stride + 1, (W + 2 * pad_l - kew) // stride + 1)
    Ho, Wo = out_hw
    wp = torch.from_numpy(pack_conv_weights(w_hwio)).to(dev)
    sc = None if scale is None else torch.as_tensor(scale, dtype=torch.float32).contiguous().to(dev)
    bi = None if bias is None else torch.as_tensor(bias, dtype=torch.float32).contiguous().to(dev)
    y = _conv_out(out, (N, Ho, Wo, cout), dev)
    rh, rw = (residual.shape[1], residual.shape[2]) if residual is not None else (0, 0)
    d = _lib.DgpConvDesc(N, H, W, Cin, cout, kh, kw, stride, rate, pad_t, pad_l, Ho, Wo, int(relu),
                         res_stride if residual is not None else 0, rh, rw)
    rng = torch.zeros((2, ABSMAX_SLOTS), dtype=torch.float32, device=dev)
    _lib.check(lib.dgp_tensor_absmax(_ptr(wp), wp.numel(), _ptr(rng[0]), _stream(dev)), "dgp_tensor_absmax")
    cells = torch.empty(wp.numel(), dtype=torch.float32, device=dev)
    if tail_slab is not None:
        _need_cuda(tail_slab, torch.float32, "tail_slab")
        _lib.check(lib.dgp_conv2d_h2_slab(C.byref(d), _ptr(x_h2), int(x_exp), _ptr(wp), _ptr(rng[0]), _ptr(sc), _ptr(bi), _ptr(residual),
                                          int(res_is_h2), int(res_exp), _ptr(y), int(y_is_h2), int(y_exp), _ptr(rng[1]), _ptr(cells),
                                          _ptr(tail_slab), tail_slab.numel() * 4, _stream(dev)), "dgp_conv2d_h2_slab")
        return y, rng[1]
    _lib.check(lib.dgp_conv2d_h2(C.byref(d), _ptr(x_h2), int(x_exp), _ptr(wp), _ptr(rng[0]), _ptr(sc), _ptr(bi), _ptr(residual),
                                 int(res_is_h2), int(res_exp), _ptr(y), int(y_is_h2), int(y_exp), _ptr(rng[1]), _ptr(cells),
                                 _stream(dev)), "dgp_conv2d_h2")
    return y, rng[1]


def f32_to_h1(x: torch.Tensor, scale_exp: int) -> torch.Tensor:
    _need_cuda(x, torch.float32, "x")
    out = torch.empty(x.shape, dtype=torch.float16, device=x.device)
    _lib.check(_lib.load().dgp_f32_to_h1(_ptr(x), x.numel(), int(scale_exp), _ptr(out), _stream(x.device)), "dgp_f32_to_h1")
    return out


def h1_to_f32(x: torch.Tensor, scale_exp: int) -> torch.Tensor:
    _need_cuda(x, torch.float16, "x")
    out = torch.empty(x.shape, dtype=torch.float32, device=x.device)
    _lib.check(_lib.load().dgp_h1_to_f32(_ptr(x), x.numel(), int(scale_exp), _ptr(out), _stream(x.device)), "dgp_h1_to_f32")
    return out


def conv2d_h1(x_h1: torch.Tensor, x_exp: int, w_hwio: np.ndarray, stride: int = 1, rate: int = 1, pad_t: int = 0, pad_l: int = 0,
              out_hw: Optional[Tuple[int, int]] = None, scale=None, bias=None, residual: Optional[torch.Tensor] = None,
              res_stride: int = 0, res_exp: int = 0, relu: bool = False, y_is_h1: bool = True, y_exp: int = 0):
    lib = _lib.load()
    _need_cuda(x_h1, torch.float16, "x_h1")
    N, H, W, Cin = x_h1.shape
    kh, kw, cin2, cout = w_hwio.shape
    assert cin2 == Cin
    dev = x_h1.device
    if out_hw is None:
        keh, kew = (kh - 1) * rate + 1, (kw - 1) * rate + 1
        out_hw = ((H + 2 * pad_t - keh) // stride + 1, (W + 2 * pad_l - kew) // stride + 1)
    Ho, Wo = out_hw
    wp = torch.from_numpy(pack_conv_weights(w_hwio)).to(dev)
    sc = None if scale is None else torch.as_tensor(scale, dtype=torch.float32).contiguous().to(dev)
    bi = None if bias is None else torch.as_tensor(bias, dtype=torch.float32).contiguous().to(dev)
    y = torch.empty((N, Ho, Wo, cout), dtype=torch.float16 if y_is_h1 else torch.float32, device=dev)
    if residual is not None:
        _need_cuda(residual, torch.float16, "residual")
    rh, rw = (residual.shape[1], residual.shape[2]) if residual is not None else (0, 0)
    d = _lib.DgpConvDesc(N, H, W, Cin, cout, kh, kw, stride, rate, pad_t, pad_l, Ho, Wo, int(relu),
                         res_stride if residual is not None else 0, rh, rw)
    rng = torch.zeros((2, ABSMAX_SLOTS), dtype=torch.float32, device=dev)
    _lib.check(lib.dgp_tensor_absmax(_ptr(wp), wp.numel(), _ptr(rng[0]), _stream(dev)), "dgp_tensor_absmax")
    cells = torch.empty(wp.numel(), dtype=torch.float16, device=dev)
    _lib.check(lib.dgp_conv2d_h1(C.byref(d), _ptr(x_h1), int(x_exp), _ptr(wp), _ptr(rng[0]), _ptr(sc), _ptr(bi), _ptr(residual),
                                 int(res_exp), _ptr(y), int(y_is_h1), int(y_exp), _ptr(rng[1]), _ptr(cells), _stream(dev)),
               "dgp_conv2d_h1")
    return y, rng[1]


def _xout_buffer(xout, shape, dt, dev) -> torch.Tensor:
    if xout is None:
        return torch.empty(shape, dtype=dt, device=dev)
    _need_cuda(xout, dt, "xout")
    assert tuple(xout.shape) == tuple(shape) and xout.is_contiguous() and xout.device == dev
    return xout


def chain_h2(r2_h2: torch.Tensor, r2_exp: int, src2_h2: torch.Tensor, src2_exp: int, w3cat: np.ndarray, scale3, bias3,
             w1: np.ndarray, scale1, bias1, res_mode: int, xout_exp: int, r1_exp: int, h1: bool = False, xout_keep: int = 1,
             xout: Optional[torch.Tensor] = None):
    lib = _lib.load()
    dt = torch.float16 if h1 else torch.float32
    _need_cuda(r2_h2, dt, "r2_h2")
    _need_cuda(src2_h2, dt, "src2_h2")
    N, Ho, Wo, Cc = r2_h2.shape
    K, C4 = w3cat.shape
    C1 = w1.shape[1]
    assert C4 == 4 * Cc and w1.shape[0] == C4
    cin2 = K - Cc
    dev = r2_h2.device
    xo = _xout_buffer(xout, (N, Ho, Wo, C4), dt, dev)
    r1 = torch.empty((N, Ho, Wo, C1), dtype=dt, device=dev)
    rng = torch.zeros((2, ABSMAX_SLOTS), dtype=torch.float32, device=dev)
    f = lambda a: None if a is None else np.ascontiguousarray(a, dtype=np.float32)
    w3c, s3, b3, w1c, s1, b1 = f(w3cat), f(scale3), f(bias3), f(w1), f(scale1), f(bias1)
    hp = lambda a: None if a is None else a.ctypes.data_as(C.c_void_p)
    args = (N, Ho, Wo, Cc, C1, cin2, int(res_mode), src2_h2.shape[1], src2_h2.shape[2], _ptr(r2_h2), int(r2_exp),
            _ptr(src2_h2), int(src2_exp), hp(w3c), hp(s3), hp(b3), hp(w1c), hp(s1), hp(b1), _ptr(xo), int(xout_exp),
            _ptr(r1), int(r1_exp), _ptr(rng[0]), _ptr(rng[1]), _stream(dev))
    if xout_keep == 1:
        _lib.check((lib.dgp_chain_h1 if h1 else lib.dgp_chain_h2)(*args), "dgp_chain_h2")
    else:
        _lib.check(lib.dgp_chain_xkeep(int(h1), int(xout_keep), *args), "dgp_chain_xkeep")
    return xo, r1, rng[0], rng[1]


def unit_h2(r1_h2: torch.Tensor, r1_exp: int, src2_h2: torch.Tensor, src2_exp: int, w2: np.ndarray, scale2, bias2, r2_exp: int,
            w3cat: np.ndarray, scale3, bias3, w1: np.ndarray, scale1, bias1, res_mode: int, xout_exp: int, r1out_exp: int, h1: bool = False,
            xout_keep: int = 1, xout: Optional[torch.Tensor] = None):
    lib = _lib.load()
    dt = torch.float16 if h1 else torch.float32
    _need_cuda(r1_h2, dt, "r1_h2")
    _need_cuda(src2_h2, dt, "src2_h2")
    N, H, W, Cc = r1_h2.shape
    K, C4 = w3cat.shape
    C1 = w1.shape[1]
    assert C4 == 4 * Cc and w1.shape[0] == C4 and w2.shape == (3, 3, Cc, Cc)
    cin2 = K - Cc
    dev = r1_h2.device
    xo = _xout_buffer(xout, (N, H, W, C4), dt, dev)
    r1o = torch.empty((N, H, W, C1), dtype=dt, device=dev)
    rng = torch.zeros((3, ABSMAX_SLOTS), dtype=torch.float32, device=dev)
    f = lambda a: None if a is None else np.ascontiguousarray(a, dtype=np.float32)
    arrs = [f(a) for a in (w2, scale2, bias2, w3cat, scale3, bias3, w1, scale1, bias1)]
    hp = lambda a: None if a is None else a.ctypes.data_as(C.c_void_p)
    args = (N, H, W, Cc, C1, cin2, int(res_mode), _ptr(r1_h2), int(r1_exp), _ptr(src2_h2), int(src2_exp),
            hp(arrs[0]), hp(arrs[1]), hp(arrs[2]), int(r2_exp), hp(arrs[3]), hp(arrs[4]), hp(arrs[5]), hp(arrs[6]),
            hp(arrs[7]), hp(arrs[8]), _ptr(xo), int(xout_exp), _ptr(r1o), int(r1out_exp), _ptr(rng[0]), _ptr(rng[1]),
            _ptr(rng[2]), _stream(dev))
    if xout_keep == 1:
        _lib.check((lib.dgp_unit_h1 if h1 else lib.dgp_unit_h2)(*args), "dgp_unit_h2")
    else:
        _lib.check(lib.dgp_unit_xkeep(int(h1), int(xout_keep), *args), "dgp_unit_xkeep")
    return xo, r1o, rng[0], rng[1], rng[2]


def maxpool_3x3s2_same(x: torch.Tensor) -> torch.Tensor:
    lib = _lib.load()
    _need_cuda(x, torch.float32, "x")
    N, H, W, Cn = x.shape
    y = torch.empty((N, (H + 1) // 2, (W + 1) // 2, Cn), dtype=torch.float32, device=x.device)
    _lib.check(lib.dgp_maxpool_3x3s2_same(_ptr(x), N, H, W, Cn, _ptr(y), _stream(x.device)), "dgp_maxpool")
    return y


def preprocess_u8(frames: torch.Tensor, mean=MEAN_PIXEL) -> torch.Tensor:
    lib = _lib.load()
    _need_cuda(frames, torch.uint8, "frames")
    out = torch.empty(tuple(frames.shape[:-1]) + (4,), dtype=torch.float32, device=frames.device)
    m = (C.c_float * 3)(*mean)
# ... 547 lines not shown
```

### include/dgp_hip.h

```cpp
#ifndef DGP_HIP_H
#define DGP_HIP_H

#include <stddef.h>
#include <stdint.h>

#ifdef __cplusplus
extern "C" {
#endif

#define DGP_ABI_VERSION 1

typedef enum dgp_status {
    DGP_OK = 0,
    DGP_ERR_INVALID = -1,
    DGP_ERR_HIP = -2,
    DGP_ERR_MISSING = -3,
    DGP_ERR_STATE = -4
} dgp_status;

typedef struct dgp_net dgp_net;

typedef struct dgp_net_desc {
    int32_t depth;
    int32_t num_joints;
// ... 138 lines not shown
                       void* stream);
int  dgp_conv2d_ranged_slab(const dgp_conv_desc* d, const float* x, const float* packed_w, const float* scale, const float* bias,
                            const float* residual, float* y, const float* x_absmax, const float* w_absmax, float* y_absmax,
                            float* tail_slab, size_t tail_slab_bytes, void* stream);
typedef struct dgp_conv_plan {
    int32_t tile;
    int32_t family;
    int32_t mode, cs, dma, deep;
    int32_t ah2, oh2, h1;
    int32_t lds;
    int32_t mtiles, ntiles, grid;
    int32_t tail_ksplit, n_main;
    int32_t st_gn, st_mc, st_mb;
    int32_t n_cu;
    char    kernel_name[32];
} dgp_conv_plan;
int  dgp_conv2d_plan(const dgp_conv_desc* d, int32_t in_fmt, int32_t out_fmt, int32_t res_fmt, int32_t have_ranges, int32_t have_cells,
                     size_t slab_bytes, int32_t force_tile, int32_t n_cu, dgp_conv_plan* out);
int    dgp_conv2d_wgrad(const dgp_conv_desc* d, const float* x, const float* dy, const float* x_absmax, const float* dy_absmax,
                        float* dw_raw, float* colsum, void* stream);
int    dgp_conv2d_wgrad_shadow(const dgp_conv_desc* d, const float* x, const float* dy, const float* x_absmax, const float* dy_absmax,
                               const float* x_prev, const float* dy_prev, void* scratch, float* dw_raw, float* colsum, void* stream);
size_t dgp_conv2d_dgrad_scratch_bytes(const dgp_conv_desc* d);
int    dgp_conv2d_dgrad(const dgp_conv_desc* d, const float* dy, const float* w_hwio, const float* scale, const float* mask,
                        const float* dx_add, int32_t add_mode, float* dx, void* scratch, int32_t ranged, void* stream);
int    dgp_h1_to_f32_pred(const void* x_h1, size_t n_halves, const float* prev, const void* gate_h1, float* out, void* stream);
int    dgp_conv2d_wgrad_h1(const dgp_conv_desc* d, const float* x, const float* dy, const float* x_absmax, const float* dy_absmax,
                           const float* x_prev, const float* dy_prev, void* scratch, float* dw_raw, float* colsum, int32_t* flag, void* stream);
int    dgp_conv2d_dgrad_h1(const dgp_conv_desc* d, const float* dy, const float* w_hwio, const float* scale, const void* gate_h1,
                           const float* dx_add, int32_t add_mode, const float* dy_prev, const float* dx_prev, const float* add_prev,
                           void* scratch, void* dx_h1, int32_t* flag, void* stream);
int    dgp_stem_wgrad_h1(const float* x_centred, const float* dpool, const float* dpool_prev, const uint8_t* idx, int32_t B, int32_t H,
                         int32_t W, int32_t H1, int32_t W1, int32_t HP, int32_t WP, void* scratch, float* dw, float* colsum, void* stream);
int    dgp_heads_backward_h1(const float* feat, const float* feat_prev, const float* dscmap, const float* dlocref, const float* dph_prev,
                             const float* w_part, const float* w_locref, const float* dfeat_prev, int32_t N, int32_t h, int32_t w,
                             int32_t Cin, int32_t nj, void* scratch, float* dw_part, float* db_part, float* dw_locref, float* db_locref,
                             void* dfeat_h1, int32_t* flag, void* stream);
int  dgp_f32_to_h2(const float* x, size_t n_floats, int32_t scale_exp, void* out, void* stream);
int  dgp_h2_to_f32(const void* x, size_t n_floats, int32_t scale_exp, float* out, void* stream);
int  dgp_conv2d_h2(const dgp_conv_desc* d, const void* x_h2, int32_t x_exp, const float* packed_w, const float* w_absmax,
                   const float* scale, const float* bias, const void* residual, int32_t res_is_h2, int32_t res_exp, void* y,
                   int32_t y_is_h2, int32_t y_exp, float* y_absmax, void* cells_scratch, void* stream);
int  dgp_conv2d_h2_slab(const dgp_conv_desc* d, const void* x_h2, int32_t x_exp, const float* packed_w, const float* w_absmax,
                        const float* scale, const float* bias, const void* residual, int32_t res_is_h2, int32_t res_exp, void* y,
                        int32_t y_is_h2, int32_t y_exp, float* y_absmax, void* cells_scratch, float* tail_slab, size_t tail_slab_bytes,
                        void* stream);
int  dgp_net_set_tier(dgp_net* net, int32_t tier);
int  dgp_net_get_tier(const dgp_net* net);
int  dgp_f32_to_h1(const float* x, size_t n_floats, int32_t scale_exp, void* out, void* stream);
int  dgp_h1_to_f32(const void* x, size_t n_floats, int32_t scale_exp, float* out, void* stream);
int  dgp_conv2d_h1(const dgp_conv_desc* d, const void* x_h1, int32_t x_exp, const float* packed_w, const float* w_absmax,
                   const float* scale, const float* bias, const void* residual_h1, int32_t res_exp, void* y,
                   int32_t y_is_h1, int32_t y_exp, float* y_absmax, void* cells_scratch, void* stream);
int  dgp_chain_h2(int32_t N, int32_t Ho, int32_t Wo, int32_t C, int32_t C1, int32_t CIN2, int32_t res_mode, int32_t res_H, int32_t res_W,
                  const void* r2_h2, int32_t r2_exp, const void* src2_h2, int32_t src2_exp,
                  const float* w3cat, const float* scale3, const float* bias3, const float* w1, const float* scale1, const float* bias1,
                  void* xout_h2, int32_t xout_exp, void* r1_h2, int32_t r1_exp, float* xout_absmax, float* r1_absmax, void* stream);
int  dgp_unit_h2(int32_t N, int32_t H, int32_t W, int32_t C, int32_t C1, int32_t CIN2, int32_t res_mode,
                 const void* r1_h2, int32_t r1_exp, const void* src2_h2, int32_t src2_exp,
                 const float* w2, const float* scale2, const float* bias2, int32_t r2_exp,
                 const float* w3cat, const float* scale3, const float* bias3, const float* w1, const float* scale1, const float* bias1,
                 void* xout_h2, int32_t xout_exp, void* r1out_h2, int32_t r1out_exp, float* r2_absmax, float* xout_absmax, float* r1_absmax,
                 void* stream);
int  dgp_chain_h1(int32_t N, int32_t Ho, int32_t Wo, int32_t C, int32_t C1, int32_t CIN2, int32_t res_mode, int32_t res_H, int32_t res_W,
                  const void* r2_h1, int32_t r2_exp, const void* src2_h1, int32_t src2_exp,
                  const float* w3cat, const float* scale3, const float* bias3, const float* w1, const float* scale1, const float* bias1,
                  void* xout_h1, int32_t xout_exp, void* r1_h1, int32_t r1_exp, float* xout_absmax, float* r1_absmax, void* stream);
int  dgp_unit_h1(int32_t N, int32_t H, int32_t W, int32_t C, int32_t C1, int32_t CIN2, int32_t res_mode,
                 const void* r1_h1, int32_t r1_exp, const void* src2_h1, int32_t src2_exp,
                 const float* w2, const float* scale2, const float* bias2, int32_t r2_exp,
                 const float* w3cat, const float* scale3, const float* bias3, const float* w1, const float* scale1, const float* bias1,
                 void* xout_h1, int32_t xout_exp, void* r1out_h1, int32_t r1out_exp, float* r2_absmax, float* xout_absmax, float* r1_absmax,
                 void* stream);
int  dgp_chain_xkeep(int32_t h1, int32_t xout_keep, int32_t N, int32_t Ho, int32_t Wo, int32_t C, int32_t C1, int32_t CIN2, int32_t res_mode,
                     int32_t res_H, int32_t res_W, const void* r2, int32_t r2_exp, const void* src2, int32_t src2_exp,
                     const float* w3cat, const float* scale3, const float* bias3, const float* w1, const float* scale1, const float* bias1,
                     void* xout, int32_t xout_exp, void* r1, int32_t r1_exp, float* xout_absmax, float* r1_absmax, void* stream);
int  dgp_unit_xkeep(int32_t h1, int32_t xout_keep, int32_t N, int32_t H, int32_t W, int32_t C, int32_t C1, int32_t CIN2, int32_t res_mode,
                    const void* r1, int32_t r1_exp, const void* src2, int32_t src2_exp,
                    const float* w2, const float* scale2, const float* bias2, int32_t r2_exp,
                    const float* w3cat, const float* scale3, const float* bias3, const float* w1, const float* scale1, const float* bias1,
                    void* xout, int32_t xout_exp, void* r1out, int32_t r1out_exp, float* r2_absmax, float* xout_absmax, float* r1_absmax,
                    void* stream);
int  dgp_net_range_status(dgp_net* net, int32_t* overflow, int32_t* calibrations, void* stream);
int  dgp_net_recalibrate(dgp_net* net);
int  dgp_net_widen(dgp_net* net);
int  dgp_net_reset_scales(dgp_net* net);
int  dgp_net_copy_scales(dgp_net* dst, const dgp_net* src, void* stream);

int  dgp_tensor_absmax(const float* x, size_t n, float* absmax_dev, void* stream);
int  dgp_maxpool_3x3s2_same(const float* x, int32_t N, int32_t H, int32_t W, int32_t C,
                            float* y, void* stream);
int  dgp_preprocess_u8(const uint8_t* frames, int64_t n_pixels, const float mean[3],
                       float* out_nhwc4, void* stream);
int  dgp_motion_energy(const uint8_t* frames, int64_t frame_bytes, int32_t n_frames, const uint8_t* prev_frame,
                       uint64_t* sums, void* stream);

typedef struct dgp_flow_params {
    double  pyr_scale;
    int32_t levels, winsize, iterations, poly_n;
    double  poly_sigma;
    int32_t flags;
} dgp_flow_params;

int  dgp_optical_flow_scratch_bytes(int32_t n_frames, int32_t H, int32_t W, const dgp_flow_params* p, size_t* bytes,
                                    int32_t* levels_used);
int  dgp_optical_flow(const uint8_t* frames, int32_t n_frames, int32_t H, int32_t W, const dgp_flow_params* p, float* flow,
                      float* magnitude, void* scratch, size_t scratch_bytes, void* stream);


int  dgp_resize_plan_size(int32_t in_size, int32_t out_size, int32_t* ksize);
int  dgp_resize_plan(int32_t in_size, int32_t out_size, int32_t* bounds, int32_t* coeffs);
int  dgp_resize_crop_u8(const uint8_t* src, int32_t B, int32_t H, int32_t W, int32_t RH, int32_t RW, const int32_t* box, uint8_t* dst,
                        const int32_t* d_plan_x, const int32_t* d_plan_y, int32_t ksize_x, int32_t ksize_y, void* stream);

enum { DGP_FILTER_BILINEAR = 2, DGP_FILTER_BICUBIC = 3, DGP_FILTER_BOX = 4 };
int  dgp_resize_plan_size_f(int32_t in_size, int32_t out_size, int32_t filter, int32_t* ksize);
int  dgp_resize_plan_f(int32_t in_size, int32_t out_size, int32_t filter, int32_t* bounds, int32_t* coeffs);
int  dgp_window_resize_u8(const uint8_t* src, int32_t src_H, int32_t src_W, int32_t x0, int32_t y0, int32_t x1, int32_t y1,
                          int32_t RH, int32_t RW, int32_t filter, int32_t mirror, uint8_t* dst, const int32_t* d_plan_x,
                          const int32_t* d_plan_y, int32_t ksize_x, int32_t ksize_y, void* stream);

int  dgp_target_maps(const double* d_entries, const int32_t* d_offsets, const double* h_entries, const int32_t* h_offsets,
                     int32_t n_frames, int32_t H, int32_t W, int32_t nj, double stride, double pos_dist_thresh, double scale,
                     double locref_stdev, int32_t weigh_only_present_joints, float* scmap, float* weights, float* lmap, float* lmask,
                     void* stream);

int  dgp_gather_frames_u8(const uint8_t* store, int64_t n_slots, int64_t slot_stride, const uint8_t* patch, int32_t m,
                          const int32_t* h_src, int32_t nt, int64_t frame_bytes, uint8_t* out, void* stream);

int  dgp_aug_affine_u8(const uint8_t* src, uint8_t* dst, int32_t H, int32_t W, const double* coef, void* stream);
int  dgp_aug_blur3_u8(const uint8_t* src, uint8_t* dst, int32_t H, int32_t W, const float* k, void* stream);
int  dgp_aug_dropout_u8(const uint8_t* src, uint8_t* dst, int32_t H, int32_t W, const uint8_t* d_mask, int32_t h, int32_t w, void* stream);
int  dgp_aug_elastic_u8(const uint8_t* src, uint8_t* dst, int32_t H, int32_t W, const float* d_field, int32_t hc, int32_t wc, void* stream);
int  dgp_aug_noise_u8(const uint8_t* src, uint8_t* dst, int32_t H, int32_t W, float scale, int32_t per_channel, uint64_t key, void* stream);

enum { DGP_JPEG_GRAY = 0, DGP_JPEG_444 = 1, DGP_JPEG_422 = 2, DGP_JPEG_420 = 3 };
typedef struct dgp_jpeg_info {
    int32_t width, height;
    int32_t ncomp;
    int32_t sampling;
    int32_t mcus_x, mcus_y;
    int32_t blocks_x[3];
    int32_t blocks_y[3];
    int32_t blocks[3];
    int32_t total_blocks;
    int32_t restart_interval;
    int32_t reserved;
    int64_t scan_offset;
} dgp_jpeg_info;
int    dgp_jpeg_probe(const uint8_t* data, int64_t n, dgp_jpeg_info* info);
int    dgp_jpeg_entropy_decode(const uint8_t* data, int64_t n, const dgp_jpeg_info* info, int16_t* coef, uint16_t* qt);
size_t dgp_jpeg_scratch_bytes(int32_t B, int32_t H, int32_t W, int32_t sampling);
int    dgp_jpeg_reconstruct_u8(const int16_t* d_coef, const uint16_t* d_qt, int32_t B, int32_t H, int32_t W, int32_t sampling, uint8_t* dst,
                               int64_t dst_frame_stride, void* scratch, size_t scratch_bytes, void* stream);

int     dgp_jpeg_quality_tables(int32_t quality, uint16_t* qt);
int64_t dgp_jpeg_encode_bound(int32_t H, int32_t W, int32_t sampling);
int     dgp_jpeg_entropy_encode(const int16_t* coef, int32_t H, int32_t W, int32_t sampling, const uint16_t* qt, uint8_t* out, int64_t cap,
                                int64_t* n);
size_t  dgp_jpeg_forward_scratch_bytes(int32_t B, int32_t H, int32_t W, int32_t sampling);
int     dgp_jpeg_forward_u8(const uint8_t* src, int32_t B, int32_t H, int32_t W, int64_t src_frame_stride, int32_t sampling,
                            const uint16_t* d_qt, const int32_t* d_markers, int32_t n_markers, int32_t dotsize, int16_t* d_coef,
                            void* scratch, size_t scratch_bytes, void* stream);

#ifdef __cplusplus
// ... 4 lines not shown
```

Baseline: 4804.

## Fuse block1 unit1 conv1 (1x1) into the stem conv+maxpool kernel

Adds a templated phase to the fused stem+pool kernel. It takes the pooled tile already held in registers, stages it through LDS, and runs the first bottleneck's 1x1 conv with MFMA, writing the r1 activations directly. This avoids a separate launch and a global re-read of the pooled activation for that conv. It is enabled by default when the net is not in calibration or tier mode, and it adds register pressure and an extra barrier phase to the stem kernel.

New measurement: 4816 (median of 6 runs). No clear change (+0.3%).

```diff
diff --git a/deepgraphpose_amd/_lib.py b/deepgraphpose_amd/_lib.py
--- a/deepgraphpose_amd/_lib.py
+++ b/deepgraphpose_amd/_lib.py
@@ -114,6 +114,7 @@
     "dgp_unit_h1": (C.c_int, [_i32] * 7 + [_vp, _i32, _vp, _i32] + [_vp] * 3 + [_i32] + [_vp] * 6 + [_vp, _i32, _vp, _i32, _vp, _vp, _vp, _vp]),
     "dgp_chain_xkeep": (C.c_int, [_i32] * 11 + [_vp, _i32, _vp, _i32] + [_vp] * 6 + [_vp, _i32, _vp, _i32, _vp, _vp, _vp]),
     "dgp_unit_xkeep": (C.c_int, [_i32] * 9 + [_vp, _i32, _vp, _i32] + [_vp] * 3 + [_i32] + [_vp] * 6 + [_vp, _i32, _vp, _i32, _vp, _vp, _vp, _vp]),
+    "dgp_root_h2": (C.c_int, [_vp, _i32, _i32, _i32] + [_vp] * 4 + [_i32] + [_vp] * 3 + [_i32] + [_vp] * 5),
     "dgp_net_range_status": (C.c_int, [_vp, C.POINTER(_i32), C.POINTER(_i32), _vp]),
     "dgp_net_recalibrate": (C.c_int, [_vp]),
     "dgp_net_reset_scales": (C.c_int, [_vp]),
diff --git a/deepgraphpose_amd/arch.py b/deepgraphpose_amd/arch.py
--- a/deepgraphpose_amd/arch.py
+++ b/deepgraphpose_amd/arch.py
@@ -92,6 +92,14 @@
     if body.endswith("/conv1+pool"):
         h1, w1 = same_out(h, 2), same_out(w, 2)
         return float(batch * h * w * 3 + elem_bytes * batch * same_out(h1, 2) * same_out(w1, 2) * 64 + 4 * 7 * 7 * 3 * 64)
+    if "/conv1+pool+" in body:
+        root, _, rest = body.partition("+pool+")
+        u0 = resnet_units(depth)[0]
+        if rest != u0.scope + "/conv1":
+            return 0.0
+        pool_px = batch * same_out(same_out(h, 2), 2) * same_out(same_out(w, 2), 2)
+        return launch_algorithmic_bytes(root + "+pool", h, w, depth, batch, elem_bytes) + \
+            elem_bytes * (pool_px * u0.depth_bottleneck + u0.depth_in * u0.depth_bottleneck)
     toks = body[5:].split("+")
     units = {u.scope: (i, u) for i, u in enumerate(resnet_units(depth))}
     plan = resnet_units(depth)
diff --git a/deepgraphpose_amd/csrc/dgp_engine.h b/deepgraphpose_amd/csrc/dgp_engine.h
--- a/deepgraphpose_amd/csrc/dgp_engine.h
+++ b/deepgraphpose_amd/csrc/dgp_engine.h
@@ -65,6 +65,7 @@
                      const float* w1, const float* sc1, const float* bi1, const float* w2 = nullptr, const float* sc2 = nullptr,
                      const float* bi2 = nullptr);
 void free_chain_plan(ChainPlan& pl);
+int build_root_conv1(const float* w1, void** d_frags, int* w_exp);
 
 constexpr size_t TAIL_SLAB_FLOATS = (size_t)512 * 128 * 128;
 
@@ -115,6 +116,8 @@
     int conv1 = -1, head_part = -1, head_locref = -1;
     std::vector<dgp::Unit> units;
     std::vector<dgp::ChainPlan> chains;
+    void* d_root_c1 = nullptr;
+    int root_c1_wexp = 0;
     bool loaded = false;
     int (*owner_sync)(void* owner, void* stream) = nullptr;
     void* owner = nullptr;
@@ -156,6 +159,7 @@
             for (void* q : {(void*)l.d_w_fused, (void*)l.d_bias_fused, l.d_wh3_fused}) if (q) (void)hipFree(q);
         }
         for (auto& c : chains) dgp::free_chain_plan(c);
+        if (d_root_c1) (void)hipFree(d_root_c1);
         for (float* q : {d_wmax, d_amax, d_inmax}) if (q) (void)hipFree(q);
         for (int* q : {d_exps, d_flag}) if (q) (void)hipFree(q);
     }
diff --git a/deepgraphpose_amd/csrc/dgp_internal.h b/deepgraphpose_amd/csrc/dgp_internal.h
--- a/deepgraphpose_amd/csrc/dgp_internal.h
+++ b/deepgraphpose_amd/csrc/dgp_internal.h
@@ -104,10 +104,16 @@
 hipError_t launch_f32_to_h2(const float* x, long long n_groups8, float scale, void* out, hipStream_t s);
 hipError_t launch_h2_to_f32(const void* x, long long n_groups8, float inv_scale, float* out, hipStream_t s);
 hipError_t launch_h2_range_check(const float* amax_slots, const int* exps, int n_layers, int* flag, hipStream_t s);
+struct RootConv1 {
+    const void* wfrag;
+    const float *bn_scale, *bn_bias;
+    float post, out_scale;
+    float* out; float* out_absmax;
+};
 hipError_t launch_stem_pool_fused(const unsigned char* frames, int B, int H, int W, const void* wcells, const float* w_absmax,
                                   const float* bn_scale, const float* bn_bias, float m0, float m1, float m2, float out_scale,
                                   float* out, float* out_absmax, hipStream_t s, int out_h1 = 0, const float* out_prev = nullptr,
-                                  unsigned char* idx = nullptr);
+                                  unsigned char* idx = nullptr, const RootConv1* c1 = nullptr);
 hipError_t launch_preprocess(const uint8_t* f, long long npix, float m0, float m1, float m2,
                              float* out, hipStream_t s);
 hipError_t launch_motion_energy(const uint8_t* frames, long long frame_bytes, int n_frames, const uint8_t* prev_frame,
diff --git a/deepgraphpose_amd/csrc/dgp_net.hip b/deepgraphpose_amd/csrc/dgp_net.hip
--- a/deepgraphpose_amd/csrc/dgp_net.hip
+++ b/deepgraphpose_amd/csrc/dgp_net.hip
@@ -125,6 +125,36 @@
     if (e == hipSuccess) e = hipMemcpy(pl.d_bi1, bi1 ? bi1 : zero.data(), C1 * sizeof(float), hipMemcpyHostToDevice);
     if (e != hipSuccess) { free_chain_plan(pl); return fail(DGP_ERR_HIP, std::string("chain plan: ") + hipGetErrorString(e)); }
     pl.ok = true;
+    return DGP_OK;
+}
+
+int build_root_conv1(const float* w1, void** d_frags, int* w_exp) {
+    constexpr int K = 64, C1 = 64, NCB = C1 / 16, NJP = K / 32;
+    const size_t chunk_f = (size_t)NCB * 512 + 256;
+    std::vector<float> src(NJP * chunk_f, 0.f);
+    float m1 = 0.f;
+    for (int i = 0; i < K * C1; ++i) m1 = std::max(m1, fabsf(w1[i]));
+    for (int jp = 0; jp < NJP; ++jp)
+        for (int cb = 0; cb < NCB; ++cb) {
+            float* f = src.data() + jp * chunk_f + (size_t)cb * 512;
+            for (int ln = 0; ln < 64; ++ln) {
+                const int g = ln >> 4, i = ln & 15, col = 32 * (cb >> 1) + 8 * (i >> 2) + 4 * (cb & 1) + (i & 3);
+                for (int j = 0; j < 8; ++j) f[ln * 8 + j] = w1[(size_t)(32 * jp + 8 * g + j) * C1 + col];
+            }
+        }
+    *w_exp = pow2_exp_for_max(m1);
+    float* d_src = nullptr;
+    if (*d_frags) { (void)hipFree(*d_frags); *d_frags = nullptr; }
+    HIP_TRY(hipMalloc(&d_src, src.size() * sizeof(float)));
+    hipError_t e = hipMemcpy(d_src, src.data(), src.size() * sizeof(float), hipMemcpyHostToDevice);
+    if (e == hipSuccess) e = hipMalloc(d_frags, (size_t)NJP * (2 * NCB + 1) * 1024);
+    if (e == hipSuccess) e = launch_chain_pack(d_src, NJP, 0, NCB, 1.f, ldexpf(1.f, *w_exp), *d_frags, nullptr);
+    if (e == hipSuccess) e = hipDeviceSynchronize();
+    (void)hipFree(d_src);
+    if (e != hipSuccess) {
+        if (*d_frags) { (void)hipFree(*d_frags); *d_frags = nullptr; }
+        return fail(DGP_ERR_HIP, std::string("root conv1 fragments: ") + hipGetErrorString(e));
+    }
     return DGP_OK;
 }
 }
@@ -493,6 +523,12 @@
         }
         if (rc2) return rc2;
     }
+    if (net->d_root_c1) { (void)hipFree(net->d_root_c1); net->d_root_c1 = nullptr; }
+    if (!net->units.empty()) {
+        const ConvLayer& l1 = net->layers[net->units[0].c1];
+        if (l1.KH == 1 && l1.KW == 1 && l1.stride == 1 && l1.Cin == 64 && l1.Cout == 64 && l1.has_bn && l1.relu && net->layers[net->conv1].Cout == 64)
+            if (int rc1 = build_root_conv1(keep_w[net->units[0].c1].data(), &net->d_root_c1, &net->root_c1_wexp)) return rc1;
+    }
     HIP_TRY(hipDeviceSynchronize());
     net->wmax_valid = true;
     net->loaded = true;
@@ -833,12 +869,28 @@
     const dgp_net_desc& d = net->desc;
     const ConvLayer& lstem = net->layers[net->conv1];
     int rc;
+    static const bool root_c1_env = (dgp_env("DGP_STEM_CONV1", 1) != 0);
+    const bool root_c1 = root_c1_env && c.stem_fused && !c.tier && !c.calib && net->d_root_c1 && !net->units.empty() && net->layers[net->units[0].c1].d_scale;
     if (c.stem_fused) {
         rc = c.layer(net->conv1, [&] {
-            ProfScope ps(net, c.s, "conv:" + lstem.scope + "+pool|stem_pool_fused", conv_flops_of(lstem, c.B * net->h1 * net->w1, false));
+            const int px1 = c.B * net->h1 * net->w1;
+            RootConv1 r1{};
+            std::string name = "conv:" + lstem.scope + "+pool|stem_pool_fused";
+            double flops = conv_flops_of(lstem, px1, false);
+            if (root_c1) {
+                const int c1 = net->units[0].c1;
+                const ConvLayer& l1 = net->layers[c1];
+                r1.wfrag = net->d_root_c1; r1.bn_scale = l1.d_scale; r1.bn_bias = l1.d_bias;
+                r1.post = ldexpf(1.f, -(net->act_exp[net->conv1] + net->root_c1_wexp)); r1.out_scale = ldexpf(1.f, net->act_exp[c1]);
+                r1.out = c.R1; r1.out_absmax = net->amax(c1);
+                name = "conv:" + lstem.scope + "+pool+" + l1.scope + "|stem_pool_fused_c1";
+                flops += conv_flops_of(l1, c.B * net->hp * net->wp, false);
+            }
+            ProfScope ps(net, c.s, name, flops);
             hipError_t e2 = launch_stem_pool_fused(c.frames, c.B, d.in_h, d.in_w, lstem.d_wh3, net->wmax(net->conv1), lstem.d_scale, lstem.d_bias,
                                                    d.mean_pixel[0], d.mean_pixel[1], d.mean_pixel[2],
-                                                   ldexpf(1.f, net->act_exp[net->conv1]), c.X[0], net->amax(net->conv1), c.s, c.tier ? 1 : 0);
+                                                   ldexpf(1.f, net->act_exp[net->conv1]), c.X[0], net->amax(net->conv1), c.s, c.tier ? 1 : 0,
+                                                   nullptr, nullptr, root_c1 ? &r1 : nullptr);
             return e2 == hipSuccess ? (int)DGP_OK : fail(DGP_ERR_HIP, std::string("stem + pool: ") + hipGetErrorString(e2));
         });
         if (rc) return rc;
@@ -861,7 +913,7 @@
         }
         if (e != hipSuccess) return fail(DGP_ERR_HIP, std::string("maxpool: ") + hipGetErrorString(e));
     }
-    c.cur = 0; c.Ra = c.R1; c.Rb = c.R2; c.r1_ready = false;
+    c.cur = 0; c.Ra = c.R1; c.Rb = c.R2; c.r1_ready = root_c1;
     c.x_rng = net->amax(net->conv1);
     c.x_exp = c.h2 ? net->act_exp[net->conv1] : 0;
     return DGP_OK;
@@ -1543,6 +1595,55 @@
     return launch_layer("dgp_unit_xkeep", io, C, C1, CIN2, res_mode, {w2, scale2, bias2, w3cat, scale3, bias3, w1, scale1, bias1}, (hipStream_t)stream);
 }
 
+int dgp_root_h2(const uint8_t* frames, int32_t B, int32_t H, int32_t W, const float* stem_w, const float* mean_pixel,
+                const float* stem_scale, const float* stem_bias, int32_t pool_exp, const float* w1, const float* scale1, const float* bias1,
+                int32_t r1_exp, void* pool_h2, void* r1_h2, float* pool_absmax, float* r1_absmax, void* stream) {
+    if (!frames || !stem_w || !mean_pixel || !pool_h2 || !pool_absmax || (w1 && (!r1_h2 || !r1_absmax)))
+        return fail(DGP_ERR_INVALID, "dgp_root_h2: null argument");
+    if (B < 1 || H < 1 || W < 1) return fail(DGP_ERR_INVALID, "dgp_root_h2: bad shape");
+    hipStream_t s = (hipStream_t)stream;
+    std::vector<float> rows((size_t)7 * 8 * 64 * 4, 0.f), rng(ABSMAX_SLOTS, 0.f), aff(4 * 64);
+    float dmean[3];
+    for (int c = 0; c < 3; ++c) dmean[c] = roundf(mean_pixel[c]) - mean_pixel[c];
+    for (int kh = 0; kh < 7; ++kh)
+        for (int kw = 0; kw < 7; ++kw)
+            for (int co = 0; co < 64; ++co) {
+                float* dst = &rows[(((size_t)(kh * 8 + kw)) * 64 + co) * 4];
+                for (int c = 0; c < 3; ++c) {
+                    dst[c] = stem_w[((size_t)(kh * 7 + kw) * 3 + c) * 64 + co];
+                    rng[0] = std::max(rng[0], fabsf(dst[c]));
+                }
+                dst[3] = dmean[0] * dst[0] + dmean[1] * dst[1] + dmean[2] * dst[2];
+            }
+    for (int c = 0; c < 64; ++c) {
+        aff[c] = stem_scale ? stem_scale[c] : 1.f; aff[64 + c] = stem_bias ? stem_bias[c] : 0.f;
+        aff[128 + c] = scale1 ? scale1[c] : 1.f; aff[192 + c] = bias1 ? bias1[c] : 0.f;
+    }
+    float *d_rows = nullptr, *d_rng = nullptr, *d_aff = nullptr;
+    void *d_cells = nullptr, *d_c1 = nullptr;
+    int w1_exp = 0, rc = DGP_OK;
+    hipError_t e = hipMalloc(&d_rows, rows.size() * sizeof(float));
+    if (e == hipSuccess) e = hipMalloc(&d_rng, rng.size() * sizeof(float));
+    if (e == hipSuccess) e = hipMalloc(&d_aff, aff.size() * sizeof(float));
+    if (e == hipSuccess) e = hipMalloc(&d_cells, rows.size() * sizeof(float));
+    if (e == hipSuccess) e = hipMemcpy(d_rows, rows.data(), rows.size() * sizeof(float), hipMemcpyHostToDevice);
+    if (e == hipSuccess) e = hipMemcpy(d_rng, rng.data(), rng.size() * sizeof(float), hipMemcpyHostToDevice);
+    if (e == hipSuccess) e = hipMemcpy(d_aff, aff.data(), aff.size() * sizeof(float), hipMemcpyHostToDevice);
+    if (e == hipSuccess) e = launch_pack_h3(d_rows, 7, 64, d_rng, d_cells, s);
+    if (e == hipSuccess && w1) rc = build_root_conv1(w1, &d_c1, &w1_exp);
+    if (e == hipSuccess && !rc) {
+        RootConv1 r1{};
+        r1.wfrag = d_c1; r1.bn_scale = d_aff + 128; r1.bn_bias = d_aff + 192;
+        r1.post = ldexpf(1.f, -(pool_exp + w1_exp)); r1.out_scale = ldexpf(1.f, r1_exp);
+        r1.out = (float*)r1_h2; r1.out_absmax = r1_absmax;
+        e = launch_stem_pool_fused(frames, B, H, W, d_cells, d_rng, d_aff, d_aff + 64, mean_pixel[0], mean_pixel[1], mean_pixel[2],
+                                   ldexpf(1.f, pool_exp), (float*)pool_h2, pool_absmax, s, 0, nullptr, nullptr, w1 ? &r1 : nullptr);
+    }
+    if (e == hipSuccess && !rc) e = hipStreamSynchronize(s);
+    for (void* q : {(void*)d_rows, (void*)d_rng, (void*)d_aff, d_cells, d_c1}) if (q) (void)hipFree(q);
+    return e != hipSuccess ? fail(DGP_ERR_HIP, std::string("dgp_root_h2: ") + hipGetErrorString(e)) : rc;
+}
+
 int dgp_net_range_status(dgp_net* net, int32_t* overflow, int32_t* calibrations, void* stream) {
     if (!net) return fail(DGP_ERR_INVALID, "dgp_net_range_status: null net");
     int flag[2] = {0, 0};
diff --git a/deepgraphpose_amd/csrc/dgp_ops.hip b/deepgraphpose_amd/csrc/dgp_ops.hip
--- a/deepgraphpose_amd/csrc/dgp_ops.hip
+++ b/deepgraphpose_amd/csrc/dgp_ops.hip
@@ -400,10 +400,16 @@
     const float* out_prev;
     unsigned char* idx;
     int B, H, W, H1, W1, HP, WP, pbh, pbw, tiles_h, tiles_w, ntiles;
+    const uint4* c1_w;
+    const float* c1_bn_scale; const float* c1_bn_bias;
+    float c1_post, c1_scale;
+    float* c1_out;
+    float* c1_absmax;
 };
 
-template <bool H1T>
+template <bool H1T, bool C1 = false>
 __global__ __launch_bounds__(512, 2) void stem_pool_fused_kernel(const StemPoolArgs p) {
+    static_assert(!(H1T && C1), "phase 5 exists in the parity instance only");
     constexpr int PH = H1T ? 3 : 5, PW = 16, SR = 2 * PH + 1, SC = 2 * PW + 1, MS = SR * SC, NRB = (MS + 15) / 16;
     constexpr int IR = 2 * SR + 5, IC = 72;
     static_assert(NRB <= 24 && NRB > 8, "one to three row blocks per wave");
@@ -435,6 +441,23 @@
         sc4[j][0] = p.bn_scale[ch] * post; bi4[j][0] = p.bn_bias[ch];
     }
     float amax = 0.f;
+    uint4 c1w[2][2][2] = {};
+    float c1sc[8] = {}, c1bi[8] = {}, amax1 = 0.f;
+    const int c1q = wave & 1;
+    if constexpr (C1) {
+        {
+#pragma unroll
+            for (int s = 0; s < 2; ++s)
+#pragma unroll
+                for (int b = 0; b < 2; ++b)
+#pragma unroll
+                    for (int pl = 0; pl < 2; ++pl) c1w[s][b][pl] = p.c1_w[(s * 9 + 2 * (2 * c1q + b) + pl) * 64 + lane];
+#pragma unroll
+            for (int k = 0; k < 8; ++k) {
+                c1sc[k] = p.c1_bn_scale[32 * c1q + 8 * g + k] * p.c1_post; c1bi[k] = p.c1_bn_bias[32 * c1q + 8 * g + k];
+            }
+        }
+    }
     constexpr int NG = IC / 4;
     static_assert(IC % 4 == 0 && IR * NG <= 512, "one group per thread");
     const int fr_r = t / NG, fr_c = 4 * (t - fr_r * NG);
@@ -557,6 +580,8 @@
             }
         }
         __syncthreads();
+        const uint4 zero4 = make_uint4(0u, 0u, 0u, 0u);
+        uint4 k0h = zero4, k0l = zero4, k1h = zero4, k1l = zero4;
         for (int q = t; q < PH * PW * 8; q += 512) {
             const int pp = q >> 3, cg = q & 7;
             const int ph = pp / PW, pw = pp - ph * PW;
@@ -628,18 +653,71 @@
                 if (!p.out_h1) dst[1] = lo;
 #pragma unroll
                 for (int k = 0; k < 8; ++k) amax = fmaxf(amax, v[k]);
+                if constexpr (C1) { if (q < 512) { k0h = hi; k0l = lo; } else { k1h = hi; k1l = lo; } }
+            }
+        }
+        if constexpr (C1) {
+            {
+                constexpr int NPX = PH * PW;
+                constexpr int XLD = 9;
+                static_assert(NPX * 8 > 512 && NPX * 8 <= 1024 && 2 * NPX * XLD * 16 <= NRB * 16 * LDC * 4, "one or two cells per thread, inside the conv1 tile");
+                uint4* sX = reinterpret_cast<uint4*>(sU);
+                asm volatile("s_waitcnt lgkmcnt(0)" ::: "memory");
+                __builtin_amdgcn_s_barrier();
+                sX[(t >> 3) * XLD + (t & 7)] = k0h; sX[(NPX + (t >> 3)) * XLD + (t & 7)] = k0l;
+                if (t < NPX * 8 - 512) {
+                    sX[(64 + (t >> 3)) * XLD + (t & 7)] = k1h; sX[(NPX + 64 + (t >> 3)) * XLD + (t & 7)] = k1l;
+                }
+                asm volatile("s_waitcnt lgkmcnt(0)" ::: "memory");
+                __builtin_amdgcn_s_barrier();
+                asm volatile("" ::: "memory");
+                for (int pb = wave >> 1; pb < PH; pb += 4) {
+                    floatx4 a1[2] = {floatx4{0.f, 0.f, 0.f, 0.f}, floatx4{0.f, 0.f, 0.f, 0.f}};
+#pragma unroll
+                    for (int s = 0; s < 2; ++s) {
+                        const uint4 xh = sX[(PW * pb + l15) * XLD + 4 * s + g], xl = sX[(NPX + PW * pb + l15) * XLD + 4 * s + g];
+#pragma unroll
+                        for (int b = 0; b < 2; ++b) {
+                            a1[b] = __builtin_amdgcn_mfma_f32_16x16x32_f16(__builtin_bit_cast(half8, c1w[s][b][1]), __builtin_bit_cast(half8, xh), a1[b], 0, 0, 0);
+                            a1[b] = __builtin_amdgcn_mfma_f32_16x16x32_f16(__builtin_bit_cast(half8, c1w[s][b][0]), __builtin_bit_cast(half8, xl), a1[b], 0, 0, 0);
+                            a1[b] = __builtin_amdgcn_mfma_f32_16x16x32_f16(__builtin_bit_cast(half8, c1w[s][b][0]), __builtin_bit_cast(half8, xh), a1[b], 0, 0, 0);
+                        }
+                    }
+                    if (ph0 + pb < p.HP && pw0 + l15 < p.WP) {
+                        float o[8];
+#pragma unroll
+                        for (int k = 0; k < 8; ++k) {
+                            o[k] = fmaxf(a1[k >> 2][k & 3] * c1sc[k] + c1bi[k], 0.f);
+                            amax1 = fmaxf(amax1, o[k]);
+                        }
+                        uint4 hi, lo;
+                        h2_pack8(o, p.c1_scale, hi, lo);
+                        const size_t cell = (((size_t)n * p.HP + ph0 + pb) * p.WP + pw0 + l15) * 8 + 4 * c1q + g;
+                        uint4* dst = reinterpret_cast<uint4*>(p.c1_out) + 2 * cell;
+                        dst[0] = hi; dst[1] = lo;
+                    }
+                }
             }
         }
         if constexpr (ALIAS) __syncthreads();
     }
     if (p.out_absmax) track_absmax(p.out_absmax, amax, lane, (int)(blockIdx.x * 8u + (threadIdx.x >> 6)));
+    if constexpr (C1) {
+        if (p.c1_absmax) track_absmax(p.c1_absmax, amax1, lane, (int)(blockIdx.x * 8u + (threadIdx.x >> 6)) + 97);
+    }
 }
 
 hipError_t launch_stem_pool_fused(const unsigned char* frames, int B, int H, int W, const void* wcells, const float* w_absmax,
                                   const float* bn_scale, const float* bn_bias, float m0, float m1, float m2, float out_scale,
-                                  float* out, float* out_absmax, hipStream_t s, int out_h1, const float* out_prev, unsigned char* idx) {
+                                  float* out, float* out_absmax, hipStream_t s, int out_h1, const float* out_prev, unsigned char* idx,
+                                  const RootConv1* c1) {
     if ((long long)B * H * W * 3 >= (1LL << 31)) return hipErrorInvalidValue;
+    if (c1 && (out_h1 || out_prev || idx || !c1->wfrag || !c1->bn_scale || !c1->bn_bias || !c1->out)) return hipErrorInvalidValue;
     StemPoolArgs a{};
+    if (c1) {
+        a.c1_w = reinterpret_cast<const uint4*>(c1->wfrag); a.c1_bn_scale = c1->bn_scale; a.c1_bn_bias = c1->bn_bias;
+        a.c1_post = c1->post; a.c1_scale = c1->out_scale; a.c1_out = c1->out; a.c1_absmax = c1->out_absmax;
+    }
     a.out_h1 = out_h1; a.out_prev = out_prev; a.idx = idx;
     a.fr_delta = (int)(reinterpret_cast<uintptr_t>(frames) & 3u); a.frames = frames - a.fr_delta; a.fr_bytes = a.fr_delta + B * H * W * 3;
     a.wcells = reinterpret_cast<const uint4*>(wcells); a.w_absmax = w_absmax; a.bn_scale = bn_scale; a.bn_bias = bn_bias;
@@ -655,7 +733,9 @@
     const int ph = h1t ? 3 : 5;
     a.tiles_h = (a.HP + ph - 1) / ph; a.tiles_w = (a.WP + 15) / 16; a.ntiles = B * a.tiles_h * a.tiles_w;
     const size_t smem = h1t ? (size_t)7 * 4 * 64 * 16 + (size_t)19 * 72 * 8 + (size_t)15 * 16 * 72 * 2 : (size_t)7 * 4 * 2 * 64 * 16 + (size_t)23 * 16 * 68 * 4;
-    const hipError_t e = h1t ? ensure_dynamic_lds<stem_pool_fused_kernel<true>>(160 * 1024) : ensure_dynamic_lds<stem_pool_fused_kernel<false>>(160 * 1024);
+    const hipError_t e = h1t  ? ensure_dynamic_lds<stem_pool_fused_kernel<true>>(160 * 1024)
+                         : c1 ? ensure_dynamic_lds<stem_pool_fused_kernel<false, true>>(160 * 1024)
+                              : ensure_dynamic_lds<stem_pool_fused_kernel<false>>(160 * 1024);
     if (e != hipSuccess) return e;
     const int n_cu = device_facts().n_cu;
     if (h1t) {
@@ -663,7 +743,8 @@
         hipLaunchKernelGGL(stem_pool_fused_kernel<true>, dim3((unsigned)grid), dim3(512), smem, s, a);
     } else {
         const int grid = a.ntiles < n_cu ? a.ntiles : n_cu;
-        hipLaunchKernelGGL(stem_pool_fused_kernel<false>, dim3((unsigned)grid), dim3(512), smem, s, a);
+        if (c1) hipLaunchKernelGGL((stem_pool_fused_kernel<false, true>), dim3((unsigned)grid), dim3(512), smem, s, a);
+        else hipLaunchKernelGGL(stem_pool_fused_kernel<false>, dim3((unsigned)grid), dim3(512), smem, s, a);
     }
     return hipGetLastError();
 }
diff --git a/deepgraphpose_amd/engine.py b/deepgraphpose_amd/engine.py
--- a/deepgraphpose_amd/engine.py
+++ b/deepgraphpose_amd/engine.py
@@ -791,6 +791,28 @@
                                  int(res_exp), _ptr(y), int(y_is_h1), int(y_exp), _ptr(rng[1]), _ptr(cells), _stream(dev)),
                "dgp_conv2d_h1")
     return y, rng[1]
+
+
+def root_h2(frames: torch.Tensor, stem_w: np.ndarray, mean_pixel, stem_scale, stem_bias, pool_exp: int, w1: Optional[np.ndarray] = None,
+            scale1=None, bias1=None, r1_exp: int = 0, r1_out: Optional[torch.Tensor] = None):
+    lib = _lib.load()
+    _need_cuda(frames, torch.uint8, "frames")
+    B, H, W, ch = frames.shape
+    assert ch == 3 and tuple(stem_w.shape) == (7, 7, 3, 64)
+    dev = frames.device
+    HP, WP = ((H + 1) // 2 + 1) // 2, ((W + 1) // 2 + 1) // 2
+    pool = torch.empty((B, HP, WP, 64), dtype=torch.float32, device=dev)
+    r1 = None
+    if w1 is not None:
+        assert tuple(w1.shape) == (64, 64)
+        r1 = _xout_buffer(r1_out, (B, HP, WP, 64), torch.float32, dev)
+    rng = torch.zeros((2, ABSMAX_SLOTS), dtype=torch.float32, device=dev)
+    f = lambda a: None if a is None else np.ascontiguousarray(a, dtype=np.float32)
+    sw, mp, ss, sb, w1c, s1, b1 = f(stem_w), f(mean_pixel), f(stem_scale), f(stem_bias), f(w1), f(scale1), f(bias1)
+    hp = lambda a: None if a is None else a.ctypes.data_as(C.c_void_p)
+    _lib.check(lib.dgp_root_h2(_ptr(frames), B, H, W, hp(sw), hp(mp), hp(ss), hp(sb), int(pool_exp), hp(w1c), hp(s1), hp(b1), int(r1_exp),
+                               _ptr(pool), _ptr(r1), _ptr(rng[0]), _ptr(rng[1]), _stream(dev)), "dgp_root_h2")
+    return pool, r1, rng[0], rng[1]
 
 
 def _xout_buffer(xout, shape, dt, dev) -> torch.Tensor:
diff --git a/include/dgp_hip.h b/include/dgp_hip.h
--- a/include/dgp_hip.h
+++ b/include/dgp_hip.h
@@ -244,6 +244,9 @@
                     const float* w3cat, const float* scale3, const float* bias3, const float* w1, const float* scale1, const float* bias1,
                     void* xout, int32_t xout_exp, void* r1out, int32_t r1out_exp, float* r2_absmax, float* xout_absmax, float* r1_absmax,
                     void* stream);
+int  dgp_root_h2(const uint8_t* frames, int32_t B, int32_t H, int32_t W, const float* stem_w, const float* mean_pixel,
+                 const float* stem_scale, const float* stem_bias, int32_t pool_exp, const float* w1, const float* scale1, const float* bias1,
+                 int32_t r1_exp, void* pool_h2, void* r1_h2, float* pool_absmax, float* r1_absmax, void* stream);
 int  dgp_net_range_status(dgp_net* net, int32_t* overflow, int32_t* calibrations, void* stream);
 int  dgp_net_recalibrate(dgp_net* net);
 int  dgp_net_widen(dgp_net* net);
```
